# DeepGraphLearning/ultra_torchdrug

Hardware: AMD Instinct MI355X
Metric: edges aggregated/sec, FB15k237-shaped 6L x 64d rspmm Bellman-Ford (predict: the reference's 18 rspmm layers per batch as 6 relation-graph + 6 entity-graph launches, tails and heads in one pass) (higher is better)
Workload: dtype f32

## Files before the change

### include/ultra_rspmm.h

```cpp
#ifndef ULTRA_RSPMM_H
#define ULTRA_RSPMM_H

#include <stddef.h>
#include <stdint.h>

#ifdef __cplusplus
extern "C" {
#endif
#pragma GCC visibility push(default)

#define ULTRA_RSPMM_ABI_VERSION 8

enum ultra_sum_op { ULTRA_SUM_ADD = 0, ULTRA_SUM_MIN = 1, ULTRA_SUM_MAX = 2 };
enum ultra_mul_op { ULTRA_MUL_MUL = 0, ULTRA_MUL_ADD = 1 };

enum ultra_status {
    ULTRA_OK = 0,
    ULTRA_ERR_BAD_OP = 1,
    ULTRA_ERR_BAD_SHAPE = 2,
    ULTRA_ERR_NULL_POINTER = 3,
    ULTRA_ERR_WORKSPACE = 4,
    ULTRA_ERR_HIP = 5,
    ULTRA_ERR_NO_DEVICE = 6,
    ULTRA_ERR_ABI = 7
// ... 99 lines not shown
int ultra_rspmm_backward_accumulate_f32(const ultra_segments *by_src_host, const ultra_segments *by_rel_host,
                                        const float *relation, const float *input, const float *output,
                                        const float *output_grad, const float *d_input_add, float *d_input,
                                        float *d_relation, void *workspace, size_t workspace_bytes, int64_t n_src,
                                        int64_t n_dst, int64_t n_rel, int64_t F, int sum_op, int mul_op, void *stream);

int ultra_rspmm_backward_active_f32(const ultra_segments *by_src, const ultra_segments *by_rel, const float *relation,
                                    const float *input, const float *output_grad, const float *d_input_add, float *d_input,
                                    float *d_relation, void *workspace, size_t workspace_bytes, int64_t n_src, int64_t n_dst,
                                    int64_t n_rel, int64_t F, int mul_op, const uint32_t *dst_active_bits, int64_t active_words,
                                    const int32_t *src_active_node, void *stream);
int ultra_node_bitmap(const int64_t *t_index, int64_t n_batch, int64_t per_row, int64_t n_node, uint32_t *bits, void *stream);

int ultra_rspmm_drelation_boundary_f32(const ultra_segments *by_rel, const int32_t *items, int64_t n_items, const int32_t *src_ptr,
                                       const int32_t *src_relpos, const int32_t *src_node, const float *input,
                                       const float *output_grad, float *d_relation, void *workspace, size_t workspace_bytes,
                                       int64_t n_src, int64_t n_rel, int64_t F, void *stream);

int ultra_rspmm_backward_weight_f32(const ultra_segments *fwd_host, const float *relation, const float *input,
                                    const float *output, const float *output_grad, float *d_weight,
                                    int64_t n_rel, int64_t F, int sum_op, int mul_op, void *stream);

int ultra_rspmm_rotate_forward_f32(const ultra_segments *fwd_host, const float *relation, const float *input,
                                   const float *add_rows, const int32_t *boundary_node, const float *boundary_value,
                                   float *out, void *workspace, size_t workspace_bytes, int64_t n_src, int64_t n_rel,
                                   int64_t F, int64_t block, int sum_op, void *stream);

int ultra_rspmm_rotate_backward_f32(const ultra_segments *by_src_host, const ultra_segments *by_rel_host,
                                    const float *relation, const float *input, const float *output,
                                    const float *output_grad, float *d_input, float *d_relation, void *workspace,
                                    size_t workspace_bytes, int64_t n_src, int64_t n_dst, int64_t n_rel, int64_t F,
                                    int64_t block, int sum_op, void *stream);

int ultra_beam_search_step_f32(const int32_t *row_ptr, const int32_t *src, const float *edge_grad, const float *input,
                               int64_t n_node, int64_t n_edges, int64_t tail, int64_t K, float *distance,
                               int32_t *back_edge, int32_t *back_rank, void *stream);


int ultra_combine_forward_f32(const float *input, const float *update, const float *weight, const float *bias,
                              const float *ln_weight, const float *ln_bias, float ln_eps, int relu, int shortcut,
                              float *out, float *z_out, int64_t rows, int64_t dim, void *stream);

int ultra_combine_forward_boundary_f32(const int32_t *boundary_node, const float *boundary_value, int64_t n_query,
                                       const float *update, const float *weight, const float *bias, const float *ln_weight,
                                       const float *ln_bias, float ln_eps, int relu, int shortcut, float *out, int64_t rows,
                                       int64_t dim, void *stream);


int ultra_combine_backward_waves(int device, int64_t rows, int *n_ln_waves, int *n_wgrad_waves);
int ultra_combine_backward_f32(const float *input, const float *update, const float *weight, const float *bias,
                               const float *ln_weight, const float *ln_bias, float ln_eps, int relu,
                               const float *grad_out, float *d_z, float *d_ln_weight_partial,
                               float *d_ln_bias_partial, float *d_weight_partial, float *d_bias_partial, int64_t rows,
                               int64_t dim, void *stream);

int ultra_combine_dxdu_f32(const float *d_z, const float *weight, const float *grad_out, float *d_input, float *d_update,
                           int64_t rows, int64_t dim, void *stream);


int ultra_combine_backward_fused_waves(int device, int64_t rows, int *n_waves);
int ultra_combine_backward_fused_f32(const float *input, const float *update, const float *weight, const float *bias,
                                     const float *ln_weight, const float *ln_bias, float ln_eps, int relu, int shortcut,
                                     const float *grad_out, const float *z, float *d_input, float *d_update, float *d_weight,
                                     float *d_bias, float *d_ln_weight, float *d_ln_bias, float *partial_workspace,
                                     size_t workspace_bytes, const int32_t *tile_list, int64_t n_list, int64_t rows, int64_t dim, void *stream);


int ultra_linear_forward_f32(const float *input, const float *weight, const float *bias, float *out, int64_t rows,
                             int64_t in_dim, int64_t out_dim, int relu, void *stream);


int ultra_score_forward_f32(const float *hidden, const float *query, const float *w1, const float *b1, const float *w2,
                            const float *b2, float *query_bias, float *out, int64_t n_node, int64_t batch, void *stream);

int ultra_relation_project_f32(const float *relation, int64_t stride_b, int64_t stride_r, const float *const *w1,
                               const float *const *b1, const float *const *w2, const float *const *b2, float *const *out,
                               int64_t n_layers, int64_t batch, int64_t repeat, int64_t n_rel, int64_t dim, void *stream);

int ultra_prepare_queries(const int64_t *batch, const float *rel_rep, int64_t stride_b, int64_t stride_r, int64_t n_batch,
                          int64_t n_rel2, int64_t n_base_rel, int64_t *anchor, int32_t *anchor32, int64_t *relation,
                          float *query, void *stream);

int ultra_relation_stack_inputs(const float *const *weights, int64_t n_layers, int64_t n_rel, int64_t n_query,
                                const int64_t *h_index, int64_t h_stride, float *tables, float *ones, int32_t *node32,
                                void *stream);

int ultra_candidate_tiles(const int64_t *t_index, int64_t n_batch, int64_t per_row, int64_t n_query, int64_t n_rows, int32_t *out,
                          void *stream);

int ultra_gather_boundary_rows_f32(const float *rows, const int32_t *node, int64_t n_query, float *out, void *stream);

int ultra_score_rows_forward_f32(const float *hidden, const float *query, const int64_t *t_index, const float *w1, const float *b1,
                                 const float *w2, const float *b2, float *h, float *in_rows, float *score, int64_t n_batch,
                                 int64_t per_row, void *stream);
int ultra_score_rows_backward_f32(const float *hidden, const float *query, const int64_t *t_index, const float *w1, const float *w2,
                                  const float *h, const float *in_rows, const float *grad, float *d_pre, float *partial,
                                  float *d_hidden, float *d_query, float *d_w1, float *d_b1, float *d_w2, float *d_b2,
                                  int64_t n_node, int64_t n_batch, int64_t per_row, void *stream);

int ultra_statistics_blocks(int64_t n_a);
int ultra_statistics_f32(const float *a, int64_t n_a, const float *b, int64_t n_b, int64_t b_repeat, double *partials,
                         float *out, void *stream);

int ultra_bce_adversarial_f32(const float *pred, int64_t rows, int64_t cols, float temperature, float *loss_rows,
                              float *dpred, void *stream);

int ultra_relation_project_backward_blocks(int device, int64_t batch, int64_t n_rel, int64_t n_layers, int64_t *blocks);
int ultra_relation_project_backward_f32(const float *relation, const float *const *w1, const float *const *b1,
                                        const float *const *w2, const float *const *grad, float *d_relation_layers,
                                        float *const *d_w1, float *const *d_b1, float *const *d_w2, float *const *d_b2,
                                        void *workspace, size_t workspace_bytes, int64_t n_layers, int64_t batch,
                                        int64_t n_rel, int64_t dim, void *stream);

int ultra_filtered_rank(const float *pred, int64_t n_query, int64_t n_cand, int64_t row_stride, const int64_t *target,
                        const int32_t *filt_ptr, const int32_t *filt_node, int64_t *rank, void *stream);


int ultra_filtered_rank_keys(const float *pred, int64_t n_query, int64_t n_cand, int64_t row_stride, const int64_t *target,
                             int64_t target_stride, const int64_t *keys, int64_t n_keys, const int64_t *anchor,
                             const int64_t *rel, int64_t index_stride, int64_t n_rel, int64_t *rank, int64_t rank_stride,
                             void *stream);
int ultra_strict_negative(const int64_t *keys, int64_t n_keys, const int64_t *anchor, const int64_t *rel, int64_t n_query,
                          int64_t n_rel, int64_t n_node, const float *rand, int64_t n_sample, int64_t *out, void *stream);
int ultra_edge_removal_weights(const ultra_segments *fwd, const ultra_segments *by_src, const ultra_segments *by_rel,
                               const int64_t *h, const int64_t *t, const int64_t *r, int64_t n_pattern,
                               int64_t n_base_rel, float *w_fwd, float *w_src, float *w_rel, int64_t slack, void *stream);
int ultra_edge_removal_marks(const ultra_segments *fwd, const ultra_segments *by_src, const ultra_segments *by_rel,
                             const int64_t *h, const int64_t *t, const int64_t *r, int64_t n_pattern, int64_t n_base_rel,
                             float *w_fwd, float *w_src, float *w_rel, int64_t slack, uint32_t *words_fwd, uint32_t *words_src,
                             uint32_t *words_rel, int64_t n_node, void *stream);


size_t ultra_relcsr_coalesce_temp_bytes(int64_t n_edges);
int ultra_relcsr_coalesce(const int64_t *row, const int64_t *col, const int64_t *rel, const float *weight,
                          int64_t n_edges, int64_t n_rows, int64_t n_cols, int64_t n_rel, int32_t *out_row,
                          int32_t *out_col, int32_t *out_rel, float *out_weight, int64_t *edge_of_input,
                          int64_t *n_unique_host, int *unit_weight_host, void *temp, size_t temp_bytes, void *stream);
size_t ultra_relcsr_plan_temp_bytes(int64_t n_edges, int64_t n_rows, int64_t piece_len);
int ultra_relcsr_plan(const int32_t *row, const int32_t *node_a, const int32_t *rel, int64_t n_edges, int64_t n_rows,
                      int64_t n_node_a, int64_t n_rel, int is_relation_plan, int wide_ids, int balance,
                      int64_t chunk_edges, int64_t chunk_rows, int64_t piece_len, int32_t *chunks,
                      int64_t cap_chunks, int32_t *long_rows, int64_t cap_long, int32_t *packed,
                      int64_t packed_slack, int64_t *counts_host, void *temp, size_t temp_bytes, void *stream);

size_t ultra_relcsr_dense_bytes(int64_t n_rows, int64_t n_cols, int kind);
int ultra_relcsr_dense(const ultra_segments *plan, int64_t n_rows, int64_t n_cols, int kind, uint32_t *dense, void *stream);

int ultra_dense_layer_supported(const ultra_segments *fwd, int64_t n_query);
int ultra_dense_layer_forward_f32(const ultra_segments *fwd, const float *relation, const float *input,
                                  const int32_t *boundary_node, const float *boundary_value, int64_t n_query, const float *weight,
                                  const float *bias, const float *ln_weight, const float *ln_bias, float ln_eps, int relu,
                                  int shortcut, float *out, void *stream);

int ultra_layer_forward_supported(const ultra_segments *fwd, int64_t n_query, int64_t n_rel);
int ultra_layer_forward_f32(const ultra_segments *fwd, const float *relation, const float *input, const int32_t *boundary_node,
                            const float *boundary_value, int64_t n_query, const float *weight, const float *bias,
                            const float *ln_weight, const float *ln_bias, float ln_eps, int relu, int shortcut, float *out,
                            int64_t n_rel, void *stream);

int ultra_second_layer_sources(const int32_t *col, int64_t n_edges, int64_t slack, const int32_t *row_list, const int32_t *list_count,
                               int64_t list_len, int64_t n_query, int64_t n_node, uint32_t *bitmap, int32_t *c_node,
                               int32_t *sources, void *stream);
int ultra_layer_forward_sources_f32(const ultra_segments *fwd, const int32_t *sources, const float *relation, const float *input,
                                    const int32_t *boundary_node, const float *boundary_value, int64_t n_query, const float *weight,
                                    const float *bias, const float *ln_weight, const float *ln_bias, float ln_eps, int relu,
                                    int shortcut, float *out, int64_t n_rel, void *stream);

int ultra_layer_score_supported(const ultra_segments *fwd, int64_t n_query, int64_t n_rel);
int ultra_layer_score_forward_f32(const ultra_segments *fwd, const float *relation, const float *input, const int32_t *boundary_node,
                                  const float *boundary_value, int64_t n_query, const float *weight, const float *bias,
                                  const float *ln_weight, const float *ln_bias, float ln_eps, int relu, int shortcut,
                                  const float *query, const float *w1, const float *b1, const float *w2, const float *b2,
                                  float *qbias, float *score, int64_t n_rel, void *stream);

int ultra_relation_graph_marks(const int32_t *head_ptr, const int32_t *head_rel, const int32_t *tail_ptr, const int32_t *tail_rel,
                               int64_t n_node, int64_t n_rel, uint8_t *marks, void *stream);

int ultra_calibrate_gather_f32(const float *table, int64_t n_rows, const int32_t *index, int64_t n_index, float *out,
                               int64_t *n_waves_host, void *stream);

#pragma GCC visibility pop
#ifdef __cplusplus
}
#endif
#endif
```

### ultra_torchdrug_amd/_lib.py

```python
import ctypes
import os

_HERE = os.path.dirname(os.path.abspath(__file__))
LIB_PATH = os.environ.get("ULTRA_RSPMM_LIB") or os.path.join(_HERE, "libultra_rspmm.so")
ABI_VERSION = 8

SUM_OPS = {"add": 0, "min": 1, "max": 2}
MUL_OPS = {"mul": 0, "add": 1}


class UltraSegments(ctypes.Structure):
    _fields_ = [
        ("struct_bytes", ctypes.c_uint32),
        ("abi_version", ctypes.c_uint32),
        ("n_rows", ctypes.c_int64),
        ("n_edges", ctypes.c_int64),
        ("row", ctypes.c_void_p),
        ("node_a", ctypes.c_void_p),
        ("node_b", ctypes.c_void_p),
        ("rel", ctypes.c_void_p),
        ("weight", ctypes.c_void_p),
        ("n_chunks", ctypes.c_int64),
        ("chunks", ctypes.c_void_p),
        ("n_long_rows", ctypes.c_int64),
        ("long_rows", ctypes.c_void_p),
        ("n_pieces", ctypes.c_int64),
        ("piece_len", ctypes.c_int64),
        ("packed", ctypes.c_void_p),
        ("packed_src_shift", ctypes.c_int64),
        ("n_hot", ctypes.c_int64),
        ("hot_nodes", ctypes.c_void_p),
        ("row_ptr", ctypes.c_void_p),
        ("dense", ctypes.c_void_p),
        ("dense_rows", ctypes.c_int64),
        ("dense_cols", ctypes.c_int64),
        ("packed_dead", ctypes.c_void_p),
    ]

    def __init__(self, *args, **kwargs):
        super().__init__(*args, **kwargs)
        if not self.struct_bytes:
            self.struct_bytes = ctypes.sizeof(type(self))
        if not self.abi_version:
            self.abi_version = ABI_VERSION


EXPORTS = (
    "ultra_rspmm_abi_version",
    "ultra_segments_bytes",
    "ultra_rspmm_status_string",
    "ultra_rspmm_last_hip_error",
    "ultra_rspmm_device_info",
    "ultra_rspmm_profile_next",
    "ultra_rspmm_event_create",
    "ultra_rspmm_event_destroy",
    "ultra_rspmm_event_elapsed_ms",
    "ultra_rspmm_force_general_path",
    "ultra_rspmm_reserve_cus",
    "ultra_rspmm_workspace_bytes",
    "ultra_rspmm_forward_f32",
    "ultra_rspmm_fwd_f32",
    "ultra_rspmm_forward_boundary_f32",
    "ultra_rspmm_frontier_f32",
    "ultra_first_layer_sparse_supported",
    "ultra_first_layer_sparse_f32",
    "ultra_rspmm_backward_boundary_rows_f32",
    "ultra_rspmm_backward_boundary_rows_workspace",
    "ultra_rspmm_backward_f32",
    "ultra_rspmm_backward_accumulate_f32",
    "ultra_rspmm_backward_weight_f32",
    "ultra_beam_search_step_f32",
    "ultra_rspmm_backward_active_f32",
    "ultra_node_bitmap",
    "ultra_rspmm_drelation_boundary_f32",
    "ultra_combine_forward_f32",
    "ultra_combine_forward_boundary_f32",
    "ultra_combine_backward_waves",
    "ultra_combine_backward_f32",
    "ultra_combine_dxdu_f32",
    "ultra_combine_backward_fused_waves",
    "ultra_combine_backward_fused_f32",
    "ultra_linear_forward_f32",
    "ultra_score_forward_f32",
    "ultra_relation_project_f32",
    "ultra_relation_project_backward_blocks",
    "ultra_relation_project_backward_f32",
    "ultra_filtered_rank",
    "ultra_filtered_rank_keys",
    "ultra_strict_negative",
    "ultra_edge_removal_weights",
    "ultra_edge_removal_marks",
    "ultra_prepare_queries",
    "ultra_relation_stack_inputs",
    "ultra_statistics_blocks",
    "ultra_statistics_f32",
    "ultra_bce_adversarial_f32",
    "ultra_candidate_tiles",
    "ultra_score_rows_forward_f32",
    "ultra_score_rows_backward_f32",
    "ultra_gather_boundary_rows_f32",
    "ultra_relcsr_coalesce_temp_bytes",
    "ultra_relcsr_coalesce",
    "ultra_relcsr_plan_temp_bytes",
    "ultra_relcsr_plan",
    "ultra_relcsr_dense_bytes",
    "ultra_relcsr_dense",
    "ultra_relation_graph_marks",
    "ultra_calibrate_gather_f32",
    "ultra_first_layer_sparse_train_f32",
    "ultra_first_layer_epilogue_backward_workspace",
    "ultra_first_layer_epilogue_backward_f32",
    "ultra_column_sum_blocks",
    "ultra_column_sum_f32",
    "ultra_dense_layer_supported",
    "ultra_dense_layer_forward_f32",
    "ultra_layer_forward_supported",
    "ultra_layer_forward_f32",
    "ultra_second_layer_sources",
    "ultra_layer_forward_sources_f32",
    "ultra_layer_score_supported",
    "ultra_layer_score_forward_f32",
    "ultra_rspmm_rotate_forward_f32",
    "ultra_rspmm_rotate_backward_f32",
)

_lib = None


class UltraLibraryError(RuntimeError):
    pass


def load():
    global _lib
    if _lib is not None:
        return _lib
    if not os.path.exists(LIB_PATH):
        raise UltraLibraryError(
            "%s not found: build it with `make -C ultra_torchdrug_amd/csrc` (hipcc --offload-arch=gfx950) or "
            "`python -c 'import __graft_entry__ as g; g.build()'`. There is no CPU/PyTorch fallback." % LIB_PATH)
    try:
        lib = ctypes.CDLL(LIB_PATH)
    except OSError as err:
        raise UltraLibraryError("cannot load %s: %s" % (LIB_PATH, err)) from err
    missing = [name for name in EXPORTS if not hasattr(lib, name)]
    if missing:
        raise UltraLibraryError("%s lacks symbols %s" % (LIB_PATH, missing))

    vp, i64, i32, sz = ctypes.c_void_p, ctypes.c_int64, ctypes.c_int, ctypes.c_size_t
    seg = ctypes.POINTER(UltraSegments)
    lib.ultra_rspmm_abi_version.restype = i32
    lib.ultra_rspmm_abi_version.argtypes = []
    lib.ultra_layer_forward_supported.restype = i32
    lib.ultra_layer_forward_supported.argtypes = [seg, i64, i64]
    lib.ultra_layer_forward_f32.restype = i32
    lib.ultra_layer_forward_f32.argtypes = [seg, vp, vp, vp, vp, i64, vp, vp, vp, vp, ctypes.c_float, i32, i32, vp, i64, vp]
    lib.ultra_second_layer_sources.restype = i32
    lib.ultra_second_layer_sources.argtypes = [vp, i64, i64, vp, vp, i64, i64, i64, vp, vp, vp, vp]
    lib.ultra_layer_forward_sources_f32.restype = i32
    lib.ultra_layer_forward_sources_f32.argtypes = [seg, vp, vp, vp, vp, vp, i64, vp, vp, vp, vp, ctypes.c_float, i32, i32, vp, i64, vp]
    lib.ultra_layer_score_supported.restype = i32
    lib.ultra_layer_score_supported.argtypes = [seg, i64, i64]
    lib.ultra_layer_score_forward_f32.restype = i32
    lib.ultra_layer_score_forward_f32.argtypes = [seg, vp, vp, vp, vp, i64, vp, vp, vp, vp, ctypes.c_float, i32, i32, vp, vp, vp, vp,
                                                  vp, vp, vp, i64, vp]
    lib.ultra_relation_graph_marks.restype = i32
    lib.ultra_relation_graph_marks.argtypes = [vp, vp, vp, vp, i64, i64, vp, vp]
    lib.ultra_segments_bytes.restype = sz
    lib.ultra_segments_bytes.argtypes = []
    lib.ultra_rspmm_status_string.restype = ctypes.c_char_p
    lib.ultra_rspmm_status_string.argtypes = [i32]
    lib.ultra_rspmm_last_hip_error.restype = i32
    lib.ultra_rspmm_last_hip_error.argtypes = []
    lib.ultra_rspmm_device_info.restype = i32
    lib.ultra_rspmm_device_info.argtypes = [i32, ctypes.POINTER(i32), ctypes.POINTER(i32), ctypes.c_char_p, sz]
    lib.ultra_rspmm_profile_next.restype = i32
    lib.ultra_rspmm_profile_next.argtypes = [vp, vp]
    lib.ultra_rspmm_event_create.restype = i32
    lib.ultra_rspmm_event_create.argtypes = [ctypes.POINTER(vp)]
    lib.ultra_rspmm_event_destroy.restype = i32
    lib.ultra_rspmm_event_destroy.argtypes = [vp]
    lib.ultra_rspmm_event_elapsed_ms.restype = i32
    lib.ultra_rspmm_event_elapsed_ms.argtypes = [vp, vp, ctypes.POINTER(ctypes.c_float)]
    lib.ultra_rspmm_force_general_path.restype = i32
    lib.ultra_rspmm_force_general_path.argtypes = [i32]
    lib.ultra_rspmm_reserve_cus.restype = i32
    lib.ultra_rspmm_reserve_cus.argtypes = [i32]
    lib.ultra_rspmm_workspace_bytes.restype = sz
    lib.ultra_rspmm_workspace_bytes.argtypes = [seg, i64]
    lib.ultra_rspmm_forward_f32.restype = i32
    lib.ultra_rspmm_forward_f32.argtypes = [seg, vp, vp, vp, vp, vp, sz, i64, i64, i64, i32, i32, vp]
    lib.ultra_rspmm_fwd_f32.restype = i32
    lib.ultra_rspmm_fwd_f32.argtypes = [vp, vp, vp, vp, vp, vp, vp, i64, i64, i64, i64, i32, i32, vp]
    lib.ultra_rspmm_forward_boundary_f32.restype = i32
    lib.ultra_rspmm_forward_boundary_f32.argtypes = [seg, vp, vp, vp, vp, i64, vp, vp, sz, i64, i64, i64, i32, i32, vp]
    lib.ultra_rspmm_backward_boundary_rows_f32.restype = i32
    lib.ultra_rspmm_backward_boundary_rows_f32.argtypes = [seg, vp, vp, vp, vp, vp, vp, sz, i64, i64, i64, i32, vp]
    lib.ultra_rspmm_backward_boundary_rows_workspace.restype = sz
    lib.ultra_rspmm_backward_boundary_rows_workspace.argtypes = [i64]
    lib.ultra_rspmm_frontier_f32.restype = i32
    lib.ultra_rspmm_frontier_f32.argtypes = [seg, vp, vp, vp, vp, vp, i64, vp, i64, i64, i64, vp]
    lib.ultra_first_layer_sparse_supported.restype = i32
    lib.ultra_first_layer_sparse_supported.argtypes = [i64, i64, i64]
    lib.ultra_first_layer_sparse_f32.restype = i32
    lib.ultra_first_layer_sparse_f32.argtypes = [seg, vp, vp, vp, vp, vp, vp, i64, vp, vp, vp, vp, ctypes.c_float, i32, i32, vp, vp, i64, i64,
                                                 vp, i64, i64, vp]
    lib.ultra_rspmm_backward_f32.restype = i32
    lib.ultra_rspmm_backward_f32.argtypes = [seg, seg, vp, vp, vp, vp, vp, vp, vp, sz, i64, i64, i64, i64, i32, i32, vp]
    lib.ultra_rspmm_backward_accumulate_f32.restype = i32
    lib.ultra_rspmm_backward_accumulate_f32.argtypes = [seg, seg, vp, vp, vp, vp, vp, vp, vp, vp, sz, i64, i64, i64, i64, i32,
                                                        i32, vp]
    lib.ultra_rspmm_backward_active_f32.restype = i32
    lib.ultra_rspmm_backward_active_f32.argtypes = [seg, seg, vp, vp, vp, vp, vp, vp, vp, sz, i64, i64, i64, i64, i32, vp, i64, vp, vp]
    lib.ultra_node_bitmap.restype = i32
    lib.ultra_node_bitmap.argtypes = [vp, i64, i64, i64, vp, vp]
    lib.ultra_rspmm_drelation_boundary_f32.restype = i32
    lib.ultra_rspmm_drelation_boundary_f32.argtypes = [seg, vp, i64, vp, vp, vp, vp, vp, vp, vp, sz, i64, i64, i64, vp]
    lib.ultra_rspmm_backward_weight_f32.restype = i32
    lib.ultra_rspmm_backward_weight_f32.argtypes = [seg, vp, vp, vp, vp, vp, i64, i64, i32, i32, vp]
    lib.ultra_beam_search_step_f32.restype = i32
    lib.ultra_beam_search_step_f32.argtypes = [vp, vp, vp, vp, i64, i64, i64, i64, vp, vp, vp, vp]
    lib.ultra_combine_forward_f32.restype = i32
    lib.ultra_combine_forward_f32.argtypes = [vp, vp, vp, vp, vp, vp, ctypes.c_float, i32, i32, vp, vp, i64, i64, vp]
    lib.ultra_combine_forward_boundary_f32.restype = i32
    lib.ultra_combine_forward_boundary_f32.argtypes = [vp, vp, i64, vp, vp, vp, vp, vp, ctypes.c_float, i32, i32, vp, i64, i64, vp]
    lib.ultra_prepare_queries.restype = i32
    lib.ultra_prepare_queries.argtypes = [vp, vp, i64, i64, i64, i64, i64, vp, vp, vp, vp, vp]
    lib.ultra_statistics_blocks.restype = i32
    lib.ultra_statistics_blocks.argtypes = [i64]
    lib.ultra_statistics_f32.restype = i32
    lib.ultra_statistics_f32.argtypes = [vp, i64, vp, i64, i64, vp, vp, vp]
    lib.ultra_gather_boundary_rows_f32.restype = i32
    lib.ultra_gather_boundary_rows_f32.argtypes = [vp, vp, i64, vp, vp]
    lib.ultra_score_rows_forward_f32.restype = i32
    lib.ultra_score_rows_forward_f32.argtypes = [vp] * 10 + [i64, i64, vp]
    lib.ultra_score_rows_backward_f32.restype = i32
    lib.ultra_score_rows_backward_f32.argtypes = [vp] * 16 + [i64, i64, i64, vp]
    lib.ultra_candidate_tiles.restype = i32
    lib.ultra_candidate_tiles.argtypes = [vp, i64, i64, i64, i64, vp, vp]
    lib.ultra_bce_adversarial_f32.restype = i32
    lib.ultra_bce_adversarial_f32.argtypes = [vp, i64, i64, ctypes.c_float, vp, vp, vp]
    lib.ultra_relation_stack_inputs.restype = i32
    lib.ultra_relation_stack_inputs.argtypes = [vp, i64, i64, i64, vp, i64, vp, vp, vp, vp]
    lib.ultra_combine_backward_waves.restype = i32
    lib.ultra_combine_backward_waves.argtypes = [i32, i64, ctypes.POINTER(i32), ctypes.POINTER(i32)]
    lib.ultra_combine_backward_f32.restype = i32
    lib.ultra_combine_backward_f32.argtypes = [vp, vp, vp, vp, vp, vp, ctypes.c_float, i32, vp, vp, vp, vp, vp, vp, i64, i64, vp]
    lib.ultra_combine_dxdu_f32.restype = i32
    lib.ultra_combine_dxdu_f32.argtypes = [vp, vp, vp, vp, vp, i64, i64, vp]
    lib.ultra_combine_backward_fused_waves.restype = i32
    lib.ultra_combine_backward_fused_waves.argtypes = [i32, i64, ctypes.POINTER(i32)]
    lib.ultra_combine_backward_fused_f32.restype = i32
    lib.ultra_combine_backward_fused_f32.argtypes = [vp, vp, vp, vp, vp, vp, ctypes.c_float, i32, i32, vp, vp, vp, vp, vp, vp, vp,
                                                     vp, vp, sz, vp, i64, i64, i64, vp]
    lib.ultra_linear_forward_f32.restype = i32
    lib.ultra_linear_forward_f32.argtypes = [vp, vp, vp, vp, i64, i64, i64, i32, vp]
    lib.ultra_score_forward_f32.restype = i32
    lib.ultra_score_forward_f32.argtypes = [vp, vp, vp, vp, vp, vp, vp, vp, i64, i64, vp]
    lib.ultra_relation_project_f32.restype = i32
    lib.ultra_relation_project_f32.argtypes = [vp, i64, i64, vp, vp, vp, vp, vp, i64, i64, i64, i64, i64, vp]
    lib.ultra_relation_project_backward_blocks.restype = i32
    lib.ultra_relation_project_backward_blocks.argtypes = [i32, i64, i64, i64, vp]
    lib.ultra_relation_project_backward_f32.restype = i32
    lib.ultra_relation_project_backward_f32.argtypes = [vp, vp, vp, vp, vp, vp, vp, vp, vp, vp, vp, sz, i64, i64, i64, i64, vp]
    lib.ultra_filtered_rank.restype = i32
    lib.ultra_filtered_rank.argtypes = [vp, i64, i64, i64, vp, vp, vp, vp, vp]
    lib.ultra_filtered_rank_keys.restype = i32
    lib.ultra_filtered_rank_keys.argtypes = [vp, i64, i64, i64, vp, i64, vp, i64, vp, vp, i64, i64, vp, i64, vp]
    lib.ultra_strict_negative.restype = i32
    lib.ultra_strict_negative.argtypes = [vp, i64, vp, vp, i64, i64, i64, vp, i64, vp, vp]
    lib.ultra_edge_removal_weights.restype = i32
    lib.ultra_edge_removal_weights.argtypes = [seg, seg, seg, vp, vp, vp, i64, i64, vp, vp, vp, i64, vp]
    lib.ultra_edge_removal_marks.restype = i32
    lib.ultra_edge_removal_marks.argtypes = [seg, seg, seg, vp, vp, vp, i64, i64, vp, vp, vp, i64, vp, vp, vp, i64, vp]
    lib.ultra_relcsr_coalesce_temp_bytes.restype = sz
    lib.ultra_relcsr_coalesce_temp_bytes.argtypes = [i64]
    lib.ultra_relcsr_coalesce.restype = i32
    lib.ultra_relcsr_coalesce.argtypes = [vp, vp, vp, vp, i64, i64, i64, i64, vp, vp, vp, vp, vp,
                                          ctypes.POINTER(i64), ctypes.POINTER(i32), vp, sz, vp]
    lib.ultra_relcsr_plan_temp_bytes.restype = sz
    lib.ultra_relcsr_plan_temp_bytes.argtypes = [i64, i64, i64]
    lib.ultra_relcsr_plan.restype = i32
    lib.ultra_relcsr_plan.argtypes = [vp, vp, vp, i64, i64, i64, i64, i32, i32, i32, i64, i64, i64, vp, i64, vp, i64,
                                      vp, i64, ctypes.POINTER(i64), vp, sz, vp]
    lib.ultra_relcsr_dense_bytes.restype = sz
    lib.ultra_relcsr_dense_bytes.argtypes = [i64, i64, i32]
    lib.ultra_relcsr_dense.restype = i32
    lib.ultra_relcsr_dense.argtypes = [seg, i64, i64, i32, vp, vp]
    lib.ultra_first_layer_sparse_train_f32.restype = i32
    lib.ultra_first_layer_sparse_train_f32.argtypes = [seg, vp, vp, vp, vp, vp, vp, i64, vp, vp, vp, vp, ctypes.c_float, i32, i32, vp, vp,
                                                       vp, i64, i64, vp, i64, i64, vp]
    lib.ultra_first_layer_epilogue_backward_workspace.restype = sz
    lib.ultra_first_layer_epilogue_backward_workspace.argtypes = [i32, i64]
    lib.ultra_first_layer_epilogue_backward_f32.restype = i32
    lib.ultra_first_layer_epilogue_backward_f32.argtypes = [vp, vp, vp, vp, vp, i64, vp, vp, vp, vp, ctypes.c_float, i32, i32, vp, vp, vp,
                                                            vp, vp, vp, vp, sz, i64, vp]
    lib.ultra_column_sum_blocks.restype = i32
    lib.ultra_column_sum_blocks.argtypes = []
    lib.ultra_column_sum_f32.restype = i32
    lib.ultra_column_sum_f32.argtypes = [vp, i64, vp, vp, vp, vp]
    lib.ultra_dense_layer_supported.restype = i32
    lib.ultra_dense_layer_supported.argtypes = [seg, i64]
    lib.ultra_dense_layer_forward_f32.restype = i32
    lib.ultra_dense_layer_forward_f32.argtypes = [seg, vp, vp, vp, vp, i64, vp, vp, vp, vp, ctypes.c_float, i32, i32, vp, vp]
    lib.ultra_calibrate_gather_f32.restype = i32
    lib.ultra_calibrate_gather_f32.argtypes = [vp, i64, vp, i64, vp, ctypes.POINTER(i64), vp]
    lib.ultra_rspmm_rotate_forward_f32.restype = i32
    lib.ultra_rspmm_rotate_forward_f32.argtypes = [seg, vp, vp, vp, vp, vp, vp, vp, sz, i64, i64, i64, i64, i32, vp]
    lib.ultra_rspmm_rotate_backward_f32.restype = i32
    lib.ultra_rspmm_rotate_backward_f32.argtypes = [seg, seg, vp, vp, vp, vp, vp, vp, vp, sz, i64, i64, i64, i64, i64, i32, vp]
    if lib.ultra_rspmm_abi_version() != ABI_VERSION:
        raise UltraLibraryError("ABI mismatch: library %d, binding %d" % (lib.ultra_rspmm_abi_version(), ABI_VERSION))
    if lib.ultra_segments_bytes() != ctypes.sizeof(UltraSegments):
        raise UltraLibraryError("struct ultra_segments: library %d bytes, binding %d bytes"
                                % (lib.ultra_segments_bytes(), ctypes.sizeof(UltraSegments)))
    _lib = lib
    return lib


def check(status):
    if status != 0:
        lib = load()
        msg = lib.ultra_rspmm_status_string(status).decode()
        if status == 5:
            msg += " [hipError_t=%d]" % lib.ultra_rspmm_last_hip_error()
        raise RuntimeError("libultra_rspmm: %s" % msg)


def device_info(device=0):
    lib = load()
    n_cu, lds = ctypes.c_int(0), ctypes.c_int(0)
    arch = ctypes.create_string_buffer(64)
    check(lib.ultra_rspmm_device_info(int(device), ctypes.byref(n_cu), ctypes.byref(lds), arch, 64))
    return {"n_cu": n_cu.value, "lds_bytes": lds.value, "arch": arch.value.decode()}
```

### ultra_torchdrug_amd/csrc/relgraph_dense.h

```cpp
#ifndef ULTRA_RELGRAPH_DENSE_H
#define ULTRA_RELGRAPH_DENSE_H

#include <hip/hip_runtime.h>

#include <cstddef>
#include <cstdint>

#include "ultra_rspmm.h"

namespace ultra_detail {

struct DenseCall {
    const ultra_segments *seg;
    int kind, sum_op, mul_op;
    const float *relation;
    const float *input;
    const float *grad;
    const float *add_rows;
    const int32_t *bnode;
    const float *bvec;
    int bdim;
    float *out;
    void *workspace;
    size_t workspace_bytes;
    int64_t gather_rows, gather2_rows, n_rel, F;
};

int persistent_cus(int *n_cu);
bool wide_groups_forced();

bool dense_applies(const DenseCall &call);
int dense_launch(const DenseCall &call, hipStream_t stream);

}

#endif
```

### ultra_torchdrug_amd/csrc/relgraph_dense.hip

```cpp
#include <hip/hip_runtime.h>

#include <cstdint>

#include "relgraph_dense.h"
#include "ultra_rspmm.h"

extern thread_local int ultra_detail_last_hip_error;

namespace {

#define HIP_TRY(expr)                                   \
    do {                                                \
        hipError_t _e = (expr);                         \
        if (_e != hipSuccess) {                         \
            ultra_detail_last_hip_error = (int)_e;      \
            (void)hipGetLastError();                    \
            return ULTRA_ERR_HIP;                       \
        }                                               \
    } while (0)

constexpr int kXcd = 8;
__device__ __forceinline__ int uniform(int v) { return __builtin_amdgcn_readfirstlane(v); }
using ultra_detail::DenseCall;
constexpr int KIND_FWD = 0, KIND_DX = 1, KIND_DREL = 2;

typedef float dn4 __attribute__((ext_vector_type(4)));
constexpr int kDnU = 8;
constexpr int kDnQ = 4;
constexpr int kDnWaves = 4;

struct DenseParams {
    const uint32_t *adj;
    const float *relation;
    const float *gather;
    const float *grad;
    const float *add_rows;
    const int32_t *bnode;
    const float *bvec;
    int bdim;
    float *out;
    long long F;
    int n_rows, n_cols, n_vt, n_ct;
    int cols_pad;
    int n_items, per_xcd;
};

__device__ __forceinline__ bool dense_item(const DenseParams &p, int &vt, int &ct) {
    const int j = blockIdx.x / kXcd;
    const int item = (blockIdx.x % kXcd) * p.per_xcd + j;
    if (j >= p.per_xcd || item >= p.n_items) return false;
    const int n_qb = (p.n_ct + kDnWaves - 1) / kDnWaves;
    vt = item / n_qb;
    ct = (item - vt * n_qb) * kDnWaves + uniform((int)(threadIdx.x >> 6));
    return ct < p.n_ct;
}

#ifndef ULTRA_DN_VARIANT
#define ULTRA_DN_VARIANT 0
#endif

template <int B>
__device__ __forceinline__ float entry(uint32_t word) {
#if ULTRA_DN_VARIANT >= 1
    return 1.0f;
#else
    return (float)((word >> (8 * B)) & 0xffu);
#endif
}

template <int MUL, bool HAS_REL>
__device__ __forceinline__ dn4 dense_rows_sum(const DenseParams &p, const int vt, const int ct, const int lane) {
    const int i = lane & 15, kq = lane >> 4;
    const long long F = p.F;
    const int col = ct * 16 + i;
    float relv = 0.0f;
    if constexpr (HAS_REL) relv = p.relation[(long long)kq * F + col];
    const uint32_t row_bytes = (uint32_t)F * 4u;
    const __amdgpu_buffer_rsrc_t rsrc_x =
        __builtin_amdgcn_make_buffer_rsrc(const_cast<float *>(p.gather), 0, (int)((uint32_t)p.n_cols * row_bytes), 0x00020000);
    const uint32_t slab_words = (uint32_t)(p.cols_pad / 4) * 64u;
    const __amdgpu_buffer_rsrc_t rsrc_a = __builtin_amdgcn_make_buffer_rsrc(
        const_cast<uint32_t *>(p.adj + (long long)vt * slab_words), 0, (int)((slab_words + 4u * 64u) * 4u), 0x00020000);
    const uint32_t voff_x0 = (uint32_t)kq * row_bytes + (uint32_t)col * 4u, voff_a = (uint32_t)lane * 4u;
    const int pick[4] = {4 * i, 4 * (i + 16), 4 * (i + 32), 4 * (i + 48)};

    auto load = [&](int u0, float (&x)[2], uint32_t (&a)[2]) {
#pragma unroll
        for (int h = 0; h < 2; ++h) {
            x[h] = __builtin_bit_cast(float, __builtin_amdgcn_raw_buffer_load_b32(rsrc_x, voff_x0 + (uint32_t)(u0 + 4 * h) * row_bytes, 0, 0));
            a[h] = __builtin_amdgcn_raw_buffer_load_b32(rsrc_a, voff_a, (uint32_t)(u0 / 4 + h) * 256u, 0);
        }
    };
    auto spread = [&](const float (&x)[2], float (&xs)[kDnU]) {
#pragma unroll
        for (int j = 0; j < kDnU; ++j) {
#if ULTRA_DN_VARIANT >= 4
            xs[j] = 1.5f;
#elif ULTRA_DN_VARIANT >= 2
            xs[j] = x[j >> 2];
#else
            xs[j] = __builtin_bit_cast(float, __builtin_amdgcn_ds_bpermute(pick[j & 3], __builtin_bit_cast(int, x[j >> 2])));
#endif
        }
    };
    dn4 acc = {0.0f, 0.0f, 0.0f, 0.0f};
    auto message = [&](float xv) -> float {
#if ULTRA_DN_VARIANT >= 3
        return xv;
#endif
        if constexpr (!HAS_REL) return xv;
        return (MUL == ULTRA_MUL_MUL) ? relv * xv : relv + xv;
    };
    auto compute = [&](const float (&xs)[kDnU], const uint32_t (&a)[2]) {
        acc = __builtin_amdgcn_mfma_f32_16x16x4f32(entry<0>(a[0]), message(xs[0]), acc, 0, 0, 0);
        acc = __builtin_amdgcn_mfma_f32_16x16x4f32(entry<1>(a[0]), message(xs[1]), acc, 0, 0, 0);
        acc = __builtin_amdgcn_mfma_f32_16x16x4f32(entry<2>(a[0]), message(xs[2]), acc, 0, 0, 0);
        acc = __builtin_amdgcn_mfma_f32_16x16x4f32(entry<3>(a[0]), message(xs[3]), acc, 0, 0, 0);
        acc = __builtin_amdgcn_mfma_f32_16x16x4f32(entry<0>(a[1]), message(xs[4]), acc, 0, 0, 0);
        acc = __builtin_amdgcn_mfma_f32_16x16x4f32(entry<1>(a[1]), message(xs[5]), acc, 0, 0, 0);
        acc = __builtin_amdgcn_mfma_f32_16x16x4f32(entry<2>(a[1]), message(xs[6]), acc, 0, 0, 0);
        acc = __builtin_amdgcn_mfma_f32_16x16x4f32(entry<3>(a[1]), message(xs[7]), acc, 0, 0, 0);
    };
    float x0[2], x1[2], s0[kDnU], s1[kDnU];
    uint32_t a0[2], a1[2], c0[2], c1[2];
    load(0, x0, a0);
    load(kDnU, x1, a1);
    spread(x0, s0);
    c0[0] = a0[0]; c0[1] = a0[1];
    for (int u0 = 0; u0 < p.cols_pad; u0 += 2 * kDnU) {
        load(u0 + 2 * kDnU, x0, a0);
        spread(x1, s1);
        c1[0] = a1[0]; c1[1] = a1[1];
        compute(s0, c0);
        load(u0 + 3 * kDnU, x1, a1);
        spread(x0, s0);
        c0[0] = a0[0]; c0[1] = a0[1];
        compute(s1, c1);
    }
    return acc;
}

template <int MUL, bool HAS_REL>
__global__ __launch_bounds__(kDnWaves * 64) void dense_rows_kernel(const DenseParams p) {
    int vt, ct;
    if (!dense_item(p, vt, ct)) return;
    const int lane = threadIdx.x & 63;
    const int i = lane & 15, kq = lane >> 4;
    const long long F = p.F;
    const int col = ct * 16 + i;
    const dn4 acc = dense_rows_sum<MUL, HAS_REL>(p, vt, ct, lane);

    int b_node = -1;
    float b_val = 0.0f;
    if (p.add_rows == nullptr && p.bnode != nullptr) {
        b_node = p.bnode[col / p.bdim];
        b_val = p.bvec[col];
    }
#pragma unroll
    for (int r = 0; r < 4; ++r) {
        const int row = vt * 16 + 4 * kq + r;
        if (row < p.n_rows) {
            float v = acc[r];
            if (p.add_rows != nullptr) v = v + p.add_rows[(long long)row * F + col];
            else if (p.bnode != nullptr) v = v + (row == b_node ? b_val : 0.0f);
            p.out[(long long)row * F + col] = v;
        }
    }
}

struct DenseLayerParams {
    DenseParams d;
    const float *weight;
    const float *bias, *gamma, *beta;
    float eps;
    int relu, shortcut;
    float *out;
};
constexpr int kDlStride = 68;

__global__ __launch_bounds__(kDnWaves * 64) void dense_layer_kernel(const DenseLayerParams q) {
    const DenseParams &p = q.d;
    __shared__ __attribute__((aligned(16))) float t_in[16 * kDlStride], t_up[16 * kDlStride], t_z[16 * kDlStride];
    int vt, ct;
    if (!dense_item(p, vt, ct)) return;
    const int lane = threadIdx.x & 63, wave = ct & 3;
    const int i = lane & 15, kq = lane >> 4;
    const long long F = p.F;
    const int col = ct * 16 + i;
    float wf[32];
    {
        const float *wrow = q.weight + (long long)(16 * wave + i) * 128 + 64 * (kq & 1) + (kq >> 1);
#pragma unroll
        for (int j = 0; j < 32; ++j) wf[j] = wrow[2 * j];
    }
    const float bias = q.bias[16 * wave + i];
    {
        const int row = vt * 16 + 4 * wave + kq;
        dn4 v = {0.0f, 0.0f, 0.0f, 0.0f};
        if (row < p.n_rows) v = *reinterpret_cast<const dn4 *>(p.gather + (long long)row * F + (ct & ~3) * 16 + 4 * i);
        *reinterpret_cast<dn4 *>(t_in + (4 * wave + kq) * kDlStride + 4 * i) = v;
    }
    const dn4 acc = dense_rows_sum<ULTRA_MUL_MUL, true>(p, vt, ct, lane);
    {
        const int b_node = p.bnode[col / 64];
        const float b_val = p.bvec[col];
#pragma unroll
        for (int r = 0; r < 4; ++r) {
            const int row = vt * 16 + 4 * kq + r;
            t_up[(4 * kq + r) * kDlStride + 16 * wave + i] = acc[r] + (row == b_node ? b_val : 0.0f);
        }
    }
    __syncthreads();
    dn4 z = {bias, bias, bias, bias};
    {
        const float *src = ((kq & 1) ? t_up : t_in) + i * kDlStride + (kq >> 1);
#pragma unroll
        for (int j = 0; j < 32; ++j) z = __builtin_amdgcn_mfma_f32_16x16x4f32(src[2 * j], wf[j], z, 0, 0, 0);
    }
#pragma unroll
    for (int r = 0; r < 4; ++r) t_z[(4 * kq + r) * kDlStride + 16 * wave + i] = z[r];
    __syncthreads();
    const int lrow = 4 * wave + kq;
    const float *zr = t_z + lrow * kDlStride;
    dn4 v = *reinterpret_cast<const dn4 *>(zr + 4 * i);
    if (q.gamma != nullptr) {
        const int half = (i >> 3) & 1;
        float s = 0.0f;
        if ((i & 7) == 0)
            for (int c = 0; c < 32; ++c) s = s + zr[32 * half + c];
        const float s0 = __shfl(s, 16 * kq, 64), s1 = __shfl(s, 16 * kq + 8, 64);
        const float mean = (s0 + s1) * (1.0f / 64.0f);
        float ss = 0.0f;
        if ((i & 7) == 0)
            for (int c = 0; c < 32; ++c) { const float dlt = zr[32 * half + c] - mean; ss = ss + dlt * dlt; }
        const float q0 = __shfl(ss, 16 * kq, 64), q1 = __shfl(ss, 16 * kq + 8, 64);
        const float var = (q0 + q1) * (1.0f / 64.0f);
        const float inv = 1.0f / sqrtf(var + q.eps);
        const dn4 g = *reinterpret_cast<const dn4 *>(q.gamma + 4 * i), b = *reinterpret_cast<const dn4 *>(q.beta + 4 * i);
        v.x = ((v.x - mean) * inv) * g.x + b.x; v.y = ((v.y - mean) * inv) * g.y + b.y;
        v.z = ((v.z - mean) * inv) * g.z + b.z; v.w = ((v.w - mean) * inv) * g.w + b.w;
    }
    if (q.relu) {
        v.x = !(v.x <= 0.0f) ? v.x : 0.0f; v.y = !(v.y <= 0.0f) ? v.y : 0.0f; v.z = !(v.z <= 0.0f) ? v.z : 0.0f; v.w = !(v.w <= 0.0f) ? v.w : 0.0f;
    }
    if (q.shortcut) {
        const dn4 x = *reinterpret_cast<const dn4 *>(t_in + lrow * kDlStride + 4 * i);
        v.x = v.x + x.x; v.y = v.y + x.y; v.z = v.z + x.z; v.w = v.w + x.w;
    }
    const int row = vt * 16 + lrow;
    if (row < p.n_rows) *reinterpret_cast<dn4 *>(q.out + (long long)row * F + (ct & ~3) * 16 + 4 * i) = v;
}

__global__ __launch_bounds__(kDnWaves * 64) void dense_drel_kernel(const DenseParams p) {
    int vt, ct;
    if (!dense_item(p, vt, ct)) return;
    const int lane = threadIdx.x & 63;
    const int i = lane & 15, kq = lane >> 4;
    const long long F = p.F;
    const int col = ct * 16 + i;
    const uint32_t row_bytes = (uint32_t)F * 4u;
    const __amdgpu_buffer_rsrc_t rsrc_x =
        __builtin_amdgcn_make_buffer_rsrc(const_cast<float *>(p.gather), 0, (int)((uint32_t)p.n_cols * row_bytes), 0x00020000);
    const uint32_t n_h = (uint32_t)p.cols_pad / 16u;
    const __amdgpu_buffer_rsrc_t rsrc_a = __builtin_amdgcn_make_buffer_rsrc(
        const_cast<uint32_t *>(p.adj), 0, (int)((4u * (uint32_t)p.n_vt * n_h + 2u) * 256u), 0x00020000);
    const uint32_t voff_a = (uint32_t)lane * 4u;
    uint32_t base_t[4];
#pragma unroll
    for (int t = 0; t < 4; ++t) base_t[t] = ((uint32_t)(t * p.n_vt + vt) * n_h) * 256u;
    const uint32_t voff_x0 = (uint32_t)kq * row_bytes + (uint32_t)col * 4u;

    auto load = [&](int h, float (&x)[kDnQ], uint32_t (&a)[4]) {
#pragma unroll
        for (int j = 0; j < kDnQ; ++j) {
            x[j] = __builtin_bit_cast(float, __builtin_amdgcn_raw_buffer_load_b32(rsrc_x, voff_x0 + (uint32_t)(16 * h + 4 * j) * row_bytes, 0, 0));
#if ULTRA_DN_VARIANT >= 4
            x[j] = 1.5f;
#endif
        }
#pragma unroll
        for (int t = 0; t < 4; ++t) a[t] = __builtin_amdgcn_raw_buffer_load_b32(rsrc_a, voff_a, base_t[t] + (uint32_t)h * 256u, 0);
    };
    dn4 acc[4];
#pragma unroll
    for (int t = 0; t < 4; ++t) acc[t] = dn4{0.0f, 0.0f, 0.0f, 0.0f};
    auto compute = [&](const float (&x)[kDnQ], const uint32_t (&a)[4]) {
#pragma unroll
        for (int t = 0; t < 4; ++t) {
            acc[t] = __builtin_amdgcn_mfma_f32_16x16x4f32(entry<0>(a[t]), x[0], acc[t], 0, 0, 0);
            acc[t] = __builtin_amdgcn_mfma_f32_16x16x4f32(entry<1>(a[t]), x[1], acc[t], 0, 0, 0);
            acc[t] = __builtin_amdgcn_mfma_f32_16x16x4f32(entry<2>(a[t]), x[2], acc[t], 0, 0, 0);
            acc[t] = __builtin_amdgcn_mfma_f32_16x16x4f32(entry<3>(a[t]), x[3], acc[t], 0, 0, 0);
        }
    };
    float xa[kDnQ], xb[kDnQ];
    uint32_t aa[4], ab[4];
    load(0, xa, aa);
    const int n_blocks = p.cols_pad / 16;
    for (int h = 0; h < n_blocks; h += 2) {
        load(h + 1, xb, ab);
        compute(xa, aa);
        load(h + 2, xa, aa);
        compute(xb, ab);
    }

    float gv[4];
#pragma unroll
    for (int r = 0; r < 4; ++r) {
        const int row = vt * 16 + 4 * kq + r;
        gv[r] = row < p.n_rows ? p.grad[(long long)row * F + col] : 0.0f;
    }
#pragma unroll
    for (int t = 0; t < 4; ++t) {
        const float q = ((gv[0] * acc[t][0] + gv[1] * acc[t][1]) + gv[2] * acc[t][2]) + gv[3] * acc[t][3];
        const int qi = __builtin_bit_cast(int, q);
        const float q0 = __builtin_bit_cast(float, __builtin_amdgcn_ds_bpermute(4 * i, qi));
        const float q1 = __builtin_bit_cast(float, __builtin_amdgcn_ds_bpermute(4 * (i + 16), qi));
        const float q2 = __builtin_bit_cast(float, __builtin_amdgcn_ds_bpermute(4 * (i + 32), qi));
        const float q3 = __builtin_bit_cast(float, __builtin_amdgcn_ds_bpermute(4 * (i + 48), qi));
        const float tile = ((q0 + q1) + q2) + q3;
        if (kq == 0) p.out[((long long)vt * 4 + t) * F + col] = tile;
    }
}

__global__ __launch_bounds__(256) void dense_drel_reduce_kernel(const float *tiles, float *d_relation, long long F, int n_vt) {
    const long long idx = (long long)blockIdx.x * blockDim.x + threadIdx.x;
    if (idx >= 4 * F) return;
    const long long t = idx / F, c = idx - t * F;
    float acc = 0.0f;
    for (int v0 = 0; v0 < n_vt; v0 += 16) {
        float part[16];
#pragma unroll
        for (int j = 0; j < 16; ++j) part[j] = tiles[((long long)min(v0 + j, n_vt - 1) * 4 + t) * F + c];
#pragma unroll
        for (int j = 0; j < 16; ++j)
            if (v0 + j < n_vt) acc = acc + part[j];
    }
    d_relation[idx] = acc;
}

__global__ __launch_bounds__(256) void dense_build_kernel(const int32_t *row, const int32_t *node_a, const int32_t *node_b,
                                                          long long n_edges, int kind, int n_vt, int cols_pad, uint8_t *dense,
                                                          const int32_t *rel) {
    const long long e = (long long)blockIdx.x * blockDim.x + threadIdx.x;
    if (e >= n_edges) return;
    long long idx;
    if (kind == 0) {
        const int v = row[e], u = node_a[e], t = rel[e];
        if (t < 0 || t >= 4) return;
        idx = ((((long long)(v >> 4) * (cols_pad / 4) + (u >> 2)) * 4 + t) * 16 + (v & 15)) * 4 + (u & 3);
    } else {
        const int t = row[e], u = node_a[e], v = node_b[e];
        if (t < 0 || t >= 4) return;
        idx = (((((long long)t * n_vt + (v >> 4)) * (cols_pad / 16) + (u >> 4)) * 4 + (u & 3)) * 16 + (v & 15)) * 4 + ((u >> 2) & 3);
    }
    dense[idx] = 1;
}

__global__ __launch_bounds__(256) void dense_zero_kernel(uint32_t *dense, long long n_words) {
    const long long k = (long long)blockIdx.x * blockDim.x + threadIdx.x;
    if (k < n_words) dense[k] = 0u;
}

inline int dense_cols_pad(long long n_cols, int kind) {
    const int round = kind == 0 ? 2 * kDnU : 8 * kDnQ;
    return (int)((n_cols + round - 1) / round * round);
}
inline long long dense_slack_bytes(int kind) { return kind == 0 ? 2 * kDnU * 64 : 2 * 256; }

}

namespace ultra_detail {

bool dense_applies(const DenseCall &c) {
    const ultra_segments *seg = c.seg;
    if (seg->dense == nullptr || seg->weight != nullptr || c.sum_op != ULTRA_SUM_ADD || c.n_rel != 4) return false;
    if (c.F % 16 != 0 || c.F * 4 >= (1LL << 24)) return false;
    if (seg->dense_cols != c.gather_rows || c.gather_rows * c.F * 4 >= (1LL << 31)) return false;
    if (c.kind == KIND_DREL) {
        if (c.mul_op != ULTRA_MUL_MUL || seg->n_rows != 4 || seg->dense_rows != c.gather2_rows) return false;
        const long long n_vt = (seg->dense_rows + 15) / 16;
        if (c.workspace == nullptr || c.workspace_bytes < (size_t)(n_vt * 4 * c.F) * sizeof(float)) return false;
    } else {
        if (seg->dense_rows != seg->n_rows) return false;
        if (c.kind == KIND_FWD && c.add_rows == nullptr && c.bnode != nullptr && c.bdim <= 0) return false;
    }
    return true;
}

int dense_launch(const DenseCall &c, hipStream_t stream) {
    const ultra_segments *seg = c.seg;
    const long long F = c.F;
    DenseParams q{};
    q.adj = seg->dense;
    q.relation = c.relation;
    q.gather = (c.kind == KIND_DX) ? c.grad : c.input;
    q.grad = c.grad;
    q.add_rows = (c.kind == KIND_DREL) ? nullptr : c.add_rows;
    q.bnode = (c.kind == KIND_FWD) ? c.bnode : nullptr;
    q.bvec = c.bvec;
    q.bdim = c.bdim;
    q.out = (c.kind == KIND_DREL) ? static_cast<float *>(c.workspace) : c.out;
    q.F = F;
    q.n_rows = (int)seg->dense_rows;
    q.n_cols = (int)seg->dense_cols;
    q.n_vt = (int)((seg->dense_rows + 15) / 16);
    q.n_ct = (int)(F / 16);
    q.cols_pad = dense_cols_pad(seg->dense_cols, c.kind == KIND_DREL ? 1 : 0);
    const int n_qb = (q.n_ct + kDnWaves - 1) / kDnWaves;
    q.n_items = q.n_vt * n_qb;
    q.per_xcd = (q.n_items + kXcd - 1) / kXcd;
    const dim3 grid((unsigned)(q.per_xcd * kXcd)), block(kDnWaves * 64);
    if (c.kind == KIND_DREL) {
        hipLaunchKernelGGL(dense_drel_kernel, grid, block, 0, stream, q);
        HIP_TRY(hipGetLastError());
        const long long n = 4 * F;
        hipLaunchKernelGGL(dense_drel_reduce_kernel, dim3((unsigned)((n + 255) / 256)), dim3(256), 0, stream,
                           static_cast<const float *>(c.workspace), c.out, F, q.n_vt);
    } else if (c.kind == KIND_FWD) {
        if (c.mul_op == ULTRA_MUL_MUL) hipLaunchKernelGGL((dense_rows_kernel<ULTRA_MUL_MUL, true>), grid, block, 0, stream, q);
        else hipLaunchKernelGGL((dense_rows_kernel<ULTRA_MUL_ADD, true>), grid, block, 0, stream, q);
    } else {
        if (c.mul_op == ULTRA_MUL_MUL) hipLaunchKernelGGL((dense_rows_kernel<ULTRA_MUL_MUL, true>), grid, block, 0, stream, q);
        else hipLaunchKernelGGL((dense_rows_kernel<ULTRA_MUL_ADD, false>), grid, block, 0, stream, q);
    }
    HIP_TRY(hipGetLastError());
    return ULTRA_OK;
}

}

namespace {

constexpr int kCalRowsPerWave = 2048;
typedef uint32_t cu4 __attribute__((ext_vector_type(4)));

__global__ __launch_bounds__(512) void calibrate_gather_kernel(const float *table, uint32_t table_bytes, const int32_t *index,
                                                               long long n_waves, float *out) {
    const int lane = threadIdx.x & 63;
    const int q = lane >> 4, j = lane & 15;
    const long long wave = ((long long)blockIdx.x * blockDim.x + threadIdx.x) >> 6;
    if (wave >= n_waves) return;
    const int32_t *mine = index + wave * kCalRowsPerWave;
    const __amdgpu_buffer_rsrc_t rsrc = __builtin_amdgcn_make_buffer_rsrc(const_cast<float *>(table), 0, (int)table_bytes, 0x00020000);
    float acc = 0.0f;
    int ids = mine[lane & 31];
    for (int k = 0; k < kCalRowsPerWave; k += 32) {
        const int nxt = (k + 32 < kCalRowsPerWave) ? mine[k + 32 + (lane & 31)] : 0;
        cu4 v[8];
#pragma unroll
        for (int u = 0; u < 8; ++u) {
            const uint32_t row = (uint32_t)__builtin_amdgcn_ds_bpermute(4 * (u * 4 + q), ids);
            v[u] = __builtin_amdgcn_raw_buffer_load_b128(rsrc, row * 256u + (uint32_t)j * 16u, 0, 0);
        }
#pragma unroll
        for (int u = 0; u < 8; ++u)
            acc += (__builtin_bit_cast(float, v[u].x) + __builtin_bit_cast(float, v[u].y)) +
                   (__builtin_bit_cast(float, v[u].z) + __builtin_bit_cast(float, v[u].w));
        ids = nxt;
    }
    out[wave * 64 + lane] = acc;
}

}

extern "C" {

size_t ultra_relcsr_dense_bytes(int64_t n_rows, int64_t n_cols, int kind) {
    if (n_rows <= 0 || n_cols <= 0 || (kind != 0 && kind != 1) || n_rows > (1 << 20) || n_cols > (1 << 20)) return 0;
    const long long n_vt = (n_rows + 15) / 16;
    const long long bytes = n_vt * 64 * dense_cols_pad(n_cols, kind) + dense_slack_bytes(kind);
    if (bytes >= (1LL << 31)) return 0;
    return (size_t)bytes;
}

int ultra_relcsr_dense(const ultra_segments *plan, int64_t n_rows, int64_t n_cols, int kind, uint32_t *dense, void *stream) {
    if (plan == nullptr) return ULTRA_ERR_NULL_POINTER;
    if (plan->struct_bytes != (uint32_t)sizeof(ultra_segments) || plan->abi_version != (uint32_t)ULTRA_RSPMM_ABI_VERSION) return ULTRA_ERR_ABI;
    if (plan->n_edges < 0 || plan->n_edges > 0x7fffffffLL) return ULTRA_ERR_BAD_SHAPE;
    if (plan->n_edges > 0 && (plan->row == nullptr || plan->node_a == nullptr || plan->rel == nullptr)) return ULTRA_ERR_NULL_POINTER;
    const size_t bytes = ultra_relcsr_dense_bytes(n_rows, n_cols, kind);
    if (bytes == 0) return ULTRA_ERR_BAD_SHAPE;
    if (dense == nullptr) return ULTRA_ERR_NULL_POINTER;
    if (plan->weight != nullptr) return ULTRA_ERR_BAD_SHAPE;
    if (kind == 0 && plan->n_rows != n_rows) return ULTRA_ERR_BAD_SHAPE;
    if (kind == 1 && (plan->n_rows != 4 || (plan->n_edges > 0 && plan->node_b == nullptr))) return ULTRA_ERR_BAD_SHAPE;
    hipStream_t s = static_cast<hipStream_t>(stream);
    const long long n_words = (long long)(bytes / 4);
    hipLaunchKernelGGL(dense_zero_kernel, dim3((unsigned)((n_words + 255) / 256)), dim3(256), 0, s, dense, n_words);
    HIP_TRY(hipGetLastError());
    if (plan->n_edges > 0) {
        hipLaunchKernelGGL(dense_build_kernel, dim3((unsigned)((plan->n_edges + 255) / 256)), dim3(256), 0, s, plan->row,
                           plan->node_a, plan->node_b, (long long)plan->n_edges, kind, (int)((n_rows + 15) / 16),
                           dense_cols_pad(n_cols, kind), reinterpret_cast<uint8_t *>(dense), plan->rel);
        HIP_TRY(hipGetLastError());
    }
    return ULTRA_OK;
}

int ultra_dense_layer_supported(const ultra_segments *fwd, int64_t n_query) {
    if (fwd == nullptr || fwd->struct_bytes != (uint32_t)sizeof(ultra_segments) || fwd->abi_version != (uint32_t)ULTRA_RSPMM_ABI_VERSION) return 0;
    if (fwd->dense == nullptr || fwd->weight != nullptr || n_query <= 0) return 0;
    if (fwd->dense_rows != fwd->n_rows || fwd->dense_rows != fwd->dense_cols) return 0;
    const long long F = n_query * 64;
    return (F * 4 < (1LL << 24) && fwd->dense_cols * F * 4 < (1LL << 31)) ? 1 : 0;
}

int ultra_dense_layer_forward_f32(const ultra_segments *fwd, const float *relation, const float *input,
                                  const int32_t *boundary_node, const float *boundary_value, int64_t n_query, const float *weight,
                                  const float *bias, const float *ln_weight, const float *ln_bias, float ln_eps, int relu,
                                  int shortcut, float *out, void *stream) {
    if (fwd != nullptr && (fwd->struct_bytes != (uint32_t)sizeof(ultra_segments) || fwd->abi_version != (uint32_t)ULTRA_RSPMM_ABI_VERSION))
        return ULTRA_ERR_ABI;
    if (!ultra_dense_layer_supported(fwd, n_query)) return ULTRA_ERR_BAD_SHAPE;
    if (relation == nullptr || input == nullptr || boundary_node == nullptr || boundary_value == nullptr || weight == nullptr ||
        bias == nullptr || out == nullptr)
        return ULTRA_ERR_NULL_POINTER;
    if (ln_weight != nullptr && ln_bias == nullptr) return ULTRA_ERR_NULL_POINTER;
    if (out == input) return ULTRA_ERR_BAD_SHAPE;
    if ((reinterpret_cast<uintptr_t>(out) | reinterpret_cast<uintptr_t>(input) | reinterpret_cast<uintptr_t>(ln_weight) |
         reinterpret_cast<uintptr_t>(ln_bias)) & 15u)
        return ULTRA_ERR_BAD_SHAPE;
    DenseLayerParams q{};
    DenseParams &d = q.d;
    const long long F = n_query * 64;
    d.adj = fwd->dense; d.relation = relation; d.gather = input; d.bnode = boundary_node; d.bvec = boundary_value; d.bdim = 64;
    d.F = F; d.n_rows = (int)fwd->dense_rows; d.n_cols = (int)fwd->dense_cols; d.n_vt = (int)((fwd->dense_rows + 15) / 16);
    d.n_ct = (int)(F / 16); d.cols_pad = dense_cols_pad(fwd->dense_cols, 0);
    d.n_items = d.n_vt * (d.n_ct / kDnWaves); d.per_xcd = (d.n_items + kXcd - 1) / kXcd;
    q.weight = weight; q.bias = bias; q.gamma = ln_weight; q.beta = ln_bias; q.eps = ln_eps; q.relu = relu; q.shortcut = shortcut;
    q.out = out;
    hipLaunchKernelGGL(dense_layer_kernel, dim3((unsigned)(d.per_xcd * kXcd)), dim3(kDnWaves * 64), 0, static_cast<hipStream_t>(stream), q);
    HIP_TRY(hipGetLastError());
    return ULTRA_OK;
}

int ultra_calibrate_gather_f32(const float *table, int64_t n_rows, const int32_t *index, int64_t n_index, float *out,
                               int64_t *n_waves_host, void *stream) {
    if (n_rows <= 0 || n_index < 0 || n_rows * 256 >= (1LL << 32)) return ULTRA_ERR_BAD_SHAPE;
    const long long n_waves = n_index / kCalRowsPerWave;
    if (n_waves_host != nullptr) *n_waves_host = n_waves;
    if (out == nullptr || n_waves == 0) return ULTRA_OK;
    if (table == nullptr || index == nullptr) return ULTRA_ERR_NULL_POINTER;
    hipLaunchKernelGGL(calibrate_gather_kernel, dim3((unsigned)((n_waves + 7) / 8)), dim3(512), 0, static_cast<hipStream_t>(stream),
                       table, (uint32_t)(n_rows * 256), index, n_waves, out);
    HIP_TRY(hipGetLastError());
    return ULTRA_OK;
}

}
```

### ultra_torchdrug_amd/csrc/rspmm_kernels.hip

```cpp
#include <hip/hip_runtime.h>
#include <type_traits>

#include <algorithm>
#include <cstdint>
#include <cstdlib>
#include <cstring>
#include <mutex>

#include "relgraph_dense.h"
#include "ultra_rspmm.h"

thread_local int ultra_detail_last_hip_error = 0;

namespace {

constexpr int kTile = 64;
#ifndef ULTRA_BLOCK
#define ULTRA_BLOCK 1024
#endif
constexpr int kBlock = ULTRA_BLOCK;
#ifndef ULTRA_UNROLL
#define ULTRA_UNROLL 8
#endif
constexpr int kUnroll = ULTRA_UNROLL;
// ... 663 lines not shown
                const int query = (int)(qq - step * (unsigned)p.rpn);
                const f32x4 zero = {0.0f, 0.0f, 0.0f, 0.0f};
                if constexpr (BND == 1) {
                    const f32x4 v = *reinterpret_cast<const f32x4 *>(bv_lds + query * 64 + c);
                    pa[q] = (node0 + step == (long long)bn_lds[query]) ? v : zero;
                } else {
                    pa[q] = (node0 + step == (long long)p.in_bnode[query]) ? *reinterpret_cast<const f32x4 *>(p.in_bvec + query * 64 + c) : zero;
                }
            }
            pb[q] = *reinterpret_cast<const f32x4 *>(p.update + gr * 64 + c);
        }
    };
    if constexpr (PF) {
        if (wave_global < n_tiles) fetch(wave_global);
    }
    for (long long t = wave_global; t < n_tiles; t += wave_total) {
        const long long row0 = t * kCbRows;
        if constexpr (!PF) fetch(t);
#pragma unroll
        for (int q = 0; q < 8; ++q) {
            const int r = 4 * q + (lane >> 4), c = (lane & 15) * 4;
            *reinterpret_cast<f32x4 *>(tile + r * kCbStride + c) = pa[q];
            *reinterpret_cast<f32x4 *>(tile + r * kCbStride + 64 + c) = pb[q];
        }
        if constexpr (PF) {
            asm volatile("s_waitcnt lgkmcnt(0)" ::: "memory");
            if (t + wave_total < n_tiles) fetch(t + wave_total);
        } else {
            asm volatile("s_waitcnt vmcnt(0) lgkmcnt(0)" ::: "memory");
        }

        f32x16 acc0, acc1;
#pragma unroll
        for (int r = 0; r < 16; ++r) { acc0[r] = bias0; acc1[r] = bias1; }
#pragma unroll
        for (int q = 0; q < 16; ++q) {
            const f32x4 av = *reinterpret_cast<const f32x4 *>(tile + i * kCbStride + 64 * h + 4 * q);
            acc0 = __builtin_amdgcn_mfma_f32_32x32x2f32(av.x, w0[4 * q + 0], acc0, 0, 0, 0);
            acc1 = __builtin_amdgcn_mfma_f32_32x32x2f32(av.x, w1[4 * q + 0], acc1, 0, 0, 0);
            acc0 = __builtin_amdgcn_mfma_f32_32x32x2f32(av.y, w0[4 * q + 1], acc0, 0, 0, 0);
            acc1 = __builtin_amdgcn_mfma_f32_32x32x2f32(av.y, w1[4 * q + 1], acc1, 0, 0, 0);
            acc0 = __builtin_amdgcn_mfma_f32_32x32x2f32(av.z, w0[4 * q + 2], acc0, 0, 0, 0);
            acc1 = __builtin_amdgcn_mfma_f32_32x32x2f32(av.z, w1[4 * q + 2], acc1, 0, 0, 0);
            acc0 = __builtin_amdgcn_mfma_f32_32x32x2f32(av.w, w0[4 * q + 3], acc0, 0, 0, 0);
            acc1 = __builtin_amdgcn_mfma_f32_32x32x2f32(av.w, w1[4 * q + 3], acc1, 0, 0, 0);
        }
        asm volatile("s_waitcnt lgkmcnt(0)" ::: "memory");

#pragma unroll
        for (int r = 0; r < 16; ++r) {
            const int row = (r & 3) + 8 * (r >> 2) + 4 * h;
            tile[row * kCbStride + 64 + i] = acc0[r];
            tile[row * kCbStride + 96 + i] = acc1[r];
        }
        asm volatile("s_waitcnt lgkmcnt(0)" ::: "memory");

        float v[32];
#pragma unroll
        for (int q = 0; q < 8; ++q) {
            const f32x4 d = *reinterpret_cast<const f32x4 *>(tile + ln_row * kCbStride + 64 + 32 * ln_half + 4 * q);
            v[4 * q + 0] = d.x; v[4 * q + 1] = d.y; v[4 * q + 2] = d.z; v[4 * q + 3] = d.w;
            if constexpr (ZOUT) {
                const long long left_z = p.rows - row0;
                const __amdgpu_buffer_rsrc_t rsrc_z = __builtin_amdgcn_make_buffer_rsrc(
                    p.z_out + row0 * 64, 0, (int)(left_z < kCbRows ? left_z : kCbRows) * 256, 0x00020000);
                __builtin_amdgcn_raw_buffer_store_b128(__builtin_bit_cast(qu4, d), rsrc_z, ln_row * 256 + ln_half * 128 + 16 * q, 0, 0);
            }
        }
        if (p.gamma != nullptr) {
            float s = 0.0f;
#pragma unroll
            for (int c = 0; c < 32; ++c) s = s + v[c];
            const float so = __shfl_xor(s, 1, 64);
            const float mean = (ln_half == 0 ? s + so : so + s) * (1.0f / 64.0f);
            float ss = 0.0f;
#pragma unroll
            for (int c = 0; c < 32; ++c) { const float dlt = v[c] - mean; ss = ss + dlt * dlt; }
            const float sso = __shfl_xor(ss, 1, 64);
            const float var = (ln_half == 0 ? ss + sso : sso + ss) * (1.0f / 64.0f);
            const float inv = 1.0f / sqrtf(var + p.eps);
#pragma unroll
            for (int q = 0; q < 8; ++q) {
                const f32x4 gq = *reinterpret_cast<const f32x4 *>(gb + 32 * ln_half + 4 * q);
                const f32x4 bq = *reinterpret_cast<const f32x4 *>(gb + 64 + 32 * ln_half + 4 * q);
                v[4 * q + 0] = ((v[4 * q + 0] - mean) * inv) * gq.x + bq.x;
                v[4 * q + 1] = ((v[4 * q + 1] - mean) * inv) * gq.y + bq.y;
                v[4 * q + 2] = ((v[4 * q + 2] - mean) * inv) * gq.z + bq.z;
                v[4 * q + 3] = ((v[4 * q + 3] - mean) * inv) * gq.w + bq.w;
            }
        }
        if (p.relu) {
#pragma unroll
            for (int c = 0; c < 32; ++c) v[c] = !(v[c] <= 0.0f) ? v[c] : 0.0f;
        }
        if (p.shortcut) {
#pragma unroll
            for (int q = 0; q < 8; ++q) {
                const f32x4 x = *reinterpret_cast<const f32x4 *>(tile + ln_row * kCbStride + 32 * ln_half + 4 * q);
                v[4 * q + 0] = v[4 * q + 0] + x.x; v[4 * q + 1] = v[4 * q + 1] + x.y;
                v[4 * q + 2] = v[4 * q + 2] + x.z; v[4 * q + 3] = v[4 * q + 3] + x.w;
            }
        }
#pragma unroll
        for (int q = 0; q < 8; ++q) {
            f32x4 d;
            d.x = v[4 * q + 0]; d.y = v[4 * q + 1]; d.z = v[4 * q + 2]; d.w = v[4 * q + 3];
            *reinterpret_cast<f32x4 *>(tile + ln_row * kCbStride + 64 + 32 * ln_half + 4 * q) = d;
        }
        asm volatile("s_waitcnt lgkmcnt(0)" ::: "memory");

        if constexpr (BND == 3) {
            if (p.rows * 256 >= (1LL << 32) - 65536) {
#pragma unroll
                for (int q = 0; q < 8; ++q) {
                    const int r = 4 * q + (lane >> 4), c = (lane & 15) * 4;
                    const f32x4 d = *reinterpret_cast<const f32x4 *>(tile + r * kCbStride + 64 + c);
                    if (rid[q] >= 0) *reinterpret_cast<f32x4 *>(p.out + (long long)rid[q] * 64 + c) = d;
                }
                asm volatile("s_waitcnt lgkmcnt(0)" ::: "memory");
                continue;
            }
            const __amdgpu_buffer_rsrc_t rsrc_all = __builtin_amdgcn_make_buffer_rsrc(p.out, 0, (int)(uint32_t)(p.rows * 256), 0x00020000);
#pragma unroll
            for (int q = 0; q < 8; ++q) {
                const int r = 4 * q + (lane >> 4), c = (lane & 15) * 4;
                const f32x4 d = *reinterpret_cast<const f32x4 *>(tile + r * kCbStride + 64 + c);
                const uint32_t off = rid[q] >= 0 ? (uint32_t)rid[q] * 256u + (uint32_t)c * 4u : 0xffffffffu;
                __builtin_amdgcn_raw_buffer_store_b128(__builtin_bit_cast(qu4, d), rsrc_all, off, 0, 0);
            }
            asm volatile("s_waitcnt lgkmcnt(0)" ::: "memory");
            continue;
        }
        const long long left = p.rows - row0;
        const __amdgpu_buffer_rsrc_t rsrc_tile = __builtin_amdgcn_make_buffer_rsrc(
            p.out + row0 * 64, 0, (int)(left < kCbRows ? left : kCbRows) * 256, 0x00020000);
#pragma unroll
        for (int q = 0; q < 8; ++q) {
            const int r = 4 * q + (lane >> 4), c = (lane & 15) * 4;
            const f32x4 d = *reinterpret_cast<const f32x4 *>(tile + r * kCbStride + 64 + c);
            __builtin_amdgcn_raw_buffer_store_b128(__builtin_bit_cast(qu4, d), rsrc_tile, r * 256 + c * 4, 0, 0);
        }
        asm volatile("s_waitcnt lgkmcnt(0)" ::: "memory");
    }
}


thread_local hipEvent_t g_prof_start = nullptr;
thread_local hipEvent_t g_prof_stop = nullptr;
bool g_force_general = false;
bool g_no_x_lds = false;
bool g_no_quad = false;
bool g_wide_groups = false;
bool g_no_dead_words = false;
#ifndef ULTRA_QUAD_U
#define ULTRA_QUAD_U 8
#endif
constexpr int kQuadU = ULTRA_QUAD_U;
#ifndef ULTRA_QUAD_UW
#define ULTRA_QUAD_UW 6
#endif
constexpr int kQuadUW = ULTRA_QUAD_UW;
#ifndef ULTRA_QUAD_UX
#define ULTRA_QUAD_UX 8
#endif
constexpr int kQuadUX = ULTRA_QUAD_UX;

#define HIP_TRY(expr)                                   \
    do {                                                \
        hipError_t _e = (expr);                         \
        if (_e != hipSuccess) {                         \
            ultra_detail_last_hip_error = (int)_e;                 \
            (void)hipGetLastError();                    \
            return ULTRA_ERR_HIP;                       \
        }                                               \
    } while (0)

struct DeviceInfo {
    bool valid = false;
    int n_cu = 0;
    int n_cu_total = 0;
    int lds_bytes = 0;
    char arch[64] = {0};
};
DeviceInfo g_dev[16];
int g_reserve_cus = 0;

int device_info(int device, DeviceInfo **out) {
    if (device < 0 || device >= 16) return ULTRA_ERR_NO_DEVICE;
    DeviceInfo &d = g_dev[device];
    if (!d.valid) {
        hipDeviceProp_t prop;
        HIP_TRY(hipGetDeviceProperties(&prop, device));
        d.n_cu_total = prop.multiProcessorCount;
        d.n_cu = std::max(kXcd, d.n_cu_total - g_reserve_cus);
        d.lds_bytes = (int)prop.maxSharedMemoryPerMultiProcessor;
        std::strncpy(d.arch, prop.gcnArchName, sizeof(d.arch) - 1);
        d.valid = true;
    }
    *out = &d;
    return ULTRA_OK;
}

int gcd_int(int a, int b) {
    while (b) {
        int t = a % b;
        a = b;
        b = t;
    }
    return a;
}

struct LdsAttrTable {
    static constexpr int kSlots = 512;
    const void *kern[kSlots];
    int dev[kSlots];
    int n = 0;
    bool seen(const void *k, int d) const {
        for (int i = 0; i < n; ++i)
            if (kern[i] == k && dev[i] == d) return true;
        return false;
    }
    void add(const void *k, int d) {
        if (n < kSlots) { kern[n] = k; dev[n] = d; ++n; }
    }
};
LdsAttrTable g_lds_attr;
std::mutex g_lds_attr_mutex;

int ensure_lds_attribute(const void *kern, size_t lds) {
    if (lds <= 48 * 1024) return ULTRA_OK;
    int dev = 0;
    HIP_TRY(hipGetDevice(&dev));
    std::lock_guard<std::mutex> lock(g_lds_attr_mutex);
    if (g_lds_attr.seen(kern, dev)) return ULTRA_OK;
    HIP_TRY(hipFuncSetAttribute(kern, hipFuncAttributeMaxDynamicSharedMemorySize, kMaxLdsBytes));
    g_lds_attr.add(kern, dev);
    return ULTRA_OK;
}

template <typename Kern, typename Params>
int launch_with_lds(Kern kern, const Params &p, int grid, size_t lds, hipStream_t stream, int block = kBlock) {
    const int rc = ensure_lds_attribute(reinterpret_cast<const void *>(kern), lds);
    if (rc) return rc;
    hipLaunchKernelGGL(kern, dim3(grid), dim3(block), lds, stream, p);
    HIP_TRY(hipGetLastError());
    return ULTRA_OK;
}

template <int KIND, int SUM, int MUL, bool UNIT_W, bool REL_LDS>
int launch_instance(const KParams &p, int grid, size_t lds, hipStream_t stream) {
    return launch_with_lds(segment_kernel<KIND, SUM, MUL, UNIT_W, REL_LDS>, p, grid, lds, stream);
}

template <int KIND, int SUM, int MUL>
int launch_wl(const KParams &p, bool unit_w, bool rel_lds, int grid, size_t lds, hipStream_t stream) {
    if constexpr (KIND == KIND_DREL) {
        if (unit_w) return launch_instance<KIND, SUM, MUL, true, false>(p, grid, kLdsHeader, stream);
        return launch_instance<KIND, SUM, MUL, false, false>(p, grid, kLdsHeader, stream);
    } else {
        if (unit_w) {
            if (rel_lds) return launch_instance<KIND, SUM, MUL, true, true>(p, grid, lds, stream);
            return launch_instance<KIND, SUM, MUL, true, false>(p, grid, lds, stream);
        }
        if (rel_lds) return launch_instance<KIND, SUM, MUL, false, true>(p, grid, lds, stream);
        return launch_instance<KIND, SUM, MUL, false, false>(p, grid, lds, stream);
    }
}

template <int KIND>
int launch_ops(const KParams &p, int sum_op, int mul_op, bool unit_w, bool rel_lds, int grid, size_t lds,
               hipStream_t stream) {
#define ULTRA_CASE(S, M)                                                    \
    if (sum_op == S && mul_op == M) return launch_wl<KIND, S, M>(p, unit_w, rel_lds, grid, lds, stream);
    ULTRA_CASE(ULTRA_SUM_ADD, ULTRA_MUL_MUL)
    ULTRA_CASE(ULTRA_SUM_ADD, ULTRA_MUL_ADD)
    ULTRA_CASE(ULTRA_SUM_MIN, ULTRA_MUL_MUL)
    ULTRA_CASE(ULTRA_SUM_MIN, ULTRA_MUL_ADD)
    ULTRA_CASE(ULTRA_SUM_MAX, ULTRA_MUL_MUL)
    ULTRA_CASE(ULTRA_SUM_MAX, ULTRA_MUL_ADD)
#undef ULTRA_CASE
    return ULTRA_ERR_BAD_OP;
}

inline bool segments_abi_ok(const ultra_segments *s) {
    return s->struct_bytes == (uint32_t)sizeof(ultra_segments) && s->abi_version == (uint32_t)ULTRA_RSPMM_ABI_VERSION;
}

int check_segments(const ultra_segments *s) {
    if (s == nullptr) return ULTRA_ERR_NULL_POINTER;
    if (!segments_abi_ok(s)) return ULTRA_ERR_ABI;
    if (s->n_rows < 0 || s->n_edges < 0 || s->n_chunks < 0 || s->n_pieces < 0 || s->n_long_rows < 0)
        return ULTRA_ERR_BAD_SHAPE;
    if (s->n_rows > 0x7fffffffLL || s->n_edges > 0x7fffffffLL || s->n_chunks > 0x7fffffffLL) return ULTRA_ERR_BAD_SHAPE;
    if (s->n_edges > 0 && (s->row == nullptr || s->node_a == nullptr || s->rel == nullptr)) return ULTRA_ERR_NULL_POINTER;
    if (s->n_chunks > 0 && s->chunks == nullptr) return ULTRA_ERR_NULL_POINTER;
    if (s->n_long_rows > 0 && s->long_rows == nullptr) return ULTRA_ERR_NULL_POINTER;
    return ULTRA_OK;
}

template <int KIND, int SUM, int MUL>
int launch_packed_w(const PParams &p, bool unit_w, int var, int grid, size_t lds, hipStream_t stream) {
#define ULTRA_VAR(V)                                                                                                  \
    if (var == V) {                                                                                                   \
        constexpr int UN = (V == 2 || V == 3) ? kUnrollBig : kUnroll;                                                 \
        if (unit_w) return launch_with_lds(packed_kernel<KIND, SUM, MUL, true, V, UN>, p, grid, lds, stream);        \
        return launch_with_lds(packed_kernel<KIND, SUM, MUL, false, V, UN>, p, grid, lds, stream);                   \
// ... 248 lines not shown
    }
    bool use_packed = false;
    if (!use_rowgroup) {
        const float *gather = (KIND == KIND_DX) ? p.grad : p.input;
        const unsigned long long gather_bytes = (unsigned long long)gather_rows * (unsigned long long)F * 4ull;
        const unsigned long long gather2_bytes = (unsigned long long)gather2_rows * (unsigned long long)F * 4ull;
        const bool big = seg->packed_src_shift >= 32;
        const bool rel_fits = lds_need <= (size_t)kMaxLdsBytes && n_rel > 0;
        const unsigned long long relation_bytes = (unsigned long long)n_rel * (unsigned long long)F * 4ull;
        const bool lds_ok = (KIND == KIND_DREL) || rel_fits || (big && relation_bytes < 0xffff0000ull && n_rel > 0);
        use_packed = !g_force_general && seg->packed != nullptr && (KIND == KIND_FWD || sum_op == ULTRA_SUM_ADD) &&
                     lds_ok && gather_bytes < 0xffff0000ull && gather2_bytes < 0xffff0000ull &&
                     (unsigned long long)F * 4ull < 0x7fffffffull && (KIND != KIND_DREL || (seg->node_b != nullptr && !big));
        if (use_packed) {
            PParams q{};
            q.meta = seg->packed;
            q.meta2 = reinterpret_cast<const uint32_t *>(big ? seg->node_a : seg->node_b);
            q.weight = seg->weight;
            q.chunks = p.chunks;
            q.relation = p.relation;
            q.gather = gather;
            q.gather2 = p.grad;
            q.add_rows = p.add_rows;
            q.bnode = p.bnode;
            q.bvec = p.bvec;
            q.bdim = p.bdim;
            q.out = p.out;
            q.partial = p.partial;
            q.F = F;
            q.gather_bytes = (uint32_t)gather_bytes;
            q.gather2_bytes = (uint32_t)gather2_bytes;
            q.relation_bytes = (uint32_t)(relation_bytes < 0xffff0000ull ? relation_bytes : 0);
            q.row_bytes = (uint32_t)(F * 4);
            q.src_shift = (uint32_t)seg->packed_src_shift;
            q.rel_mask = big ? 0xffffff00u : ((1u << (seg->packed_src_shift - 8)) - 1u) << 8;
            q.n_chunks = p.n_chunks;
            q.n_rel = p.n_rel;
            q.n_tiles = n_tiles;
            q.split = split;
            q.n_slots = p.n_slots;
            q.blocks_per_label = blocks_per_label;
            const bool needs_rel = (KIND == KIND_FWD) || (KIND == KIND_DX && mul_op == ULTRA_MUL_MUL);
            const size_t lds_x_bytes = (size_t)gather_rows * kTile * sizeof(float);
            int var = 0;
            size_t lds_bytes = needs_rel ? lds_need : 0;
            if (big) {
                var = (needs_rel && !rel_fits) ? 2 : 3;
                if (var == 2) lds_bytes = 0;
            } else if (seg->n_hot > 0) {
                const size_t hot_bytes = (size_t)seg->n_hot * kTile * sizeof(float);
                if (lds_bytes + hot_bytes > (size_t)kMaxLdsBytes) return ULTRA_ERR_BAD_SHAPE;
                var = 4;
                lds_bytes += hot_bytes;
                q.hot_nodes = seg->hot_nodes;
                q.n_hot = (int)seg->n_hot;
            } else if ((KIND != KIND_DREL || mul_op == ULTRA_MUL_MUL) && !g_no_x_lds && gather_rows > 0 &&
                       lds_bytes + lds_x_bytes <= (size_t)kMaxLdsBytes) {
                var = 1;
                lds_bytes += lds_x_bytes;
            }
            q.n_gather_rows = (int)gather_rows;
            auto aligned16 = [](const void *ptr) { return (reinterpret_cast<uintptr_t>(ptr) & 15u) == 0; };
            const unsigned long long meta_bytes = ((unsigned long long)seg->n_edges + 16ull) * 4ull;
            q.meta_bytes = (uint32_t)(meta_bytes < 0xffff0000ull ? meta_bytes : 0);
            q.meta2_bytes = (uint32_t)((unsigned long long)seg->n_edges * 4ull);
            const unsigned long long out_bytes = (unsigned long long)seg->n_rows * (unsigned long long)F * 4ull;
            q.out_bytes = (uint32_t)(out_bytes < 0xffff0000ull ? out_bytes : 0);
            const bool quad = !g_no_quad && (var == 0 || var == 1) && (F % 4) == 0 && q.out_bytes != 0 &&
                              q.meta_bytes != 0 && (unsigned long long)F * 4ull < (1ull << 24) &&
                              (KIND != KIND_DREL || gather2_rows < (1ll << 24)) && aligned16(gather) && aligned16(p.grad) &&
                              aligned16(p.out) && aligned16(p.add_rows) && aligned16(p.partial) && aligned16(p.bvec) &&
                              (p.bnode == nullptr || p.bdim % 4 == 0);
            if (quad) {
                const int slots_per_label = (q.n_slots + kXcd - 1) / kXcd;
                int conc = 1;
                while (!g_no_concurrent_tiles && conc * 2 <= slots_per_label && blocks_per_label % (conc * 2) == 0 &&
                       blocks_per_label / (conc * 2) >= 4)
                    conc *= 2;
                if (const char *force = getenv("ULTRA_CONC")) {
                    const int want = atoi(force);
                    const char *min_rows = getenv("ULTRA_CONC_MIN_ROWS");
                    if (want >= 1 && blocks_per_label % want == 0 && (min_rows == nullptr || gather_rows >= atoll(min_rows)))
                        conc = want;
                }
                q.concurrent = conc;
                size_t act_bytes = 0;
                if (KIND == KIND_DREL && var == 0 && F % kTile == 0) {
                    if (p.act_bits != nullptr && p.act_words > 0 && lds_bytes + (size_t)p.act_words * 4 <= (size_t)kMaxLdsBytes) {
                        q.act_bits = p.act_bits;
                        q.act_words = p.act_words;
                        act_bytes = (size_t)p.act_words * 4;
                    } else if (KIND == KIND_DREL && p.act_node != nullptr && mul_op == ULTRA_MUL_MUL) {
                        q.act_node = p.act_node;
                    }
                }
                const bool dead = seg->packed_dead != nullptr && !g_no_dead_words && var == 0 && q.act_node == nullptr &&
                                  sum_op == ULTRA_SUM_ADD && mul_op == ULTRA_MUL_MUL;
                if (dead) { q.meta = seg->packed_dead; q.weight = nullptr; }
                rc = launch_quad<KIND>(q, sum_op, mul_op, dead || seg->weight == nullptr, var == 1, grid,
                                       kLdsHeader + lds_bytes + act_bytes, stream, dead);
            }
            if (!quad) rc = launch_packed<KIND>(q, sum_op, mul_op, seg->weight == nullptr, var, grid, kLdsHeader + lds_bytes, stream);
            if (rc) return rc;
        }
    }
    if (!use_packed && !use_rowgroup) {
        rc = launch_ops<KIND>(p, sum_op, mul_op, seg->weight == nullptr, rel_lds, grid,
                              kLdsHeader + (rel_lds ? lds_need : 0), stream);
        if (rc) return rc;
    }
    if (ev_stop != nullptr) HIP_TRY(stamp(ev_stop));

    if (seg->n_long_rows > 0) {
        FixParams fp;
        fp.long_rows = seg->long_rows;
        fp.partial = p.partial;
        fp.add_rows = p.add_rows;
        fp.bnode = p.bnode;
        fp.bvec = p.bvec;
        fp.bdim = p.bdim;
        fp.out = p.out;
        fp.F = F;
        fp.n_long = (int)seg->n_long_rows;
        fp.n_tiles = n_tiles;
        const long long waves = (long long)fp.n_long * n_tiles;
        const int fgrid = (int)((waves + 3) / 4);
        const int red = (KIND == KIND_FWD) ? sum_op : ULTRA_SUM_ADD;
        const bool many_pieces = seg->n_pieces >= 128 * seg->n_long_rows;
        if (red == ULTRA_SUM_ADD && many_pieces)
            hipLaunchKernelGGL((fixup_kernel<ULTRA_SUM_ADD, 64>), dim3(fgrid), dim3(256), 0, stream, fp);
        else if (red == ULTRA_SUM_ADD) hipLaunchKernelGGL(fixup_kernel<ULTRA_SUM_ADD>, dim3(fgrid), dim3(256), 0, stream, fp);
        else if (red == ULTRA_SUM_MIN) hipLaunchKernelGGL(fixup_kernel<ULTRA_SUM_MIN>, dim3(fgrid), dim3(256), 0, stream, fp);
        else hipLaunchKernelGGL(fixup_kernel<ULTRA_SUM_MAX>, dim3(fgrid), dim3(256), 0, stream, fp);
        HIP_TRY(hipGetLastError());
    }
    return ULTRA_OK;
}

#include "rotate.inc"

}

namespace ultra_detail {
int persistent_cus(int *n_cu) {
    int dev = 0;
    HIP_TRY(hipGetDevice(&dev));
    DeviceInfo *di = nullptr;
    const int rc = device_info(dev, &di);
    if (rc) return rc;
    *n_cu = di->n_cu;
    return ULTRA_OK;
}
bool wide_groups_forced() { return g_wide_groups; }
}

extern "C" {

int ultra_rspmm_abi_version(void) { return ULTRA_RSPMM_ABI_VERSION; }

size_t ultra_segments_bytes(void) { return sizeof(ultra_segments); }

const char *ultra_rspmm_status_string(int status) {
    switch (status) {
        case ULTRA_OK: return "ok";
        case ULTRA_ERR_BAD_OP: return "unknown sum/mul operator code";
        case ULTRA_ERR_BAD_SHAPE: return "bad shape (negative size, F <= 0 or index range beyond int32)";
        case ULTRA_ERR_NULL_POINTER: return "required pointer is NULL";
        case ULTRA_ERR_WORKSPACE: return "workspace is NULL or smaller than ultra_rspmm_workspace_bytes()";
        case ULTRA_ERR_HIP: return "HIP runtime error (see ultra_rspmm_last_hip_error)";
        case ULTRA_ERR_NO_DEVICE: return "no usable HIP device";
        case ULTRA_ERR_ABI: return "ultra_segments.struct_bytes / abi_version are not this library's (binding written against another include/ultra_rspmm.h)";
        default: return "unknown status";
    }
}

int ultra_rspmm_last_hip_error(void) { return ultra_detail_last_hip_error; }

int ultra_rspmm_reserve_cus(int n) {
    if (n < 0) return ULTRA_ERR_BAD_SHAPE;
    g_reserve_cus = n;
    for (DeviceInfo &d : g_dev)
        if (d.valid) d.n_cu = std::max(kXcd, d.n_cu_total - n);
    return ULTRA_OK;
}

int ultra_rspmm_device_info(int device, int *n_cu, int *lds_bytes, char *arch_host, size_t arch_len) {
    DeviceInfo *di = nullptr;
    int rc = device_info(device, &di);
    if (rc) return rc;
    if (n_cu) *n_cu = di->n_cu_total;
    if (lds_bytes) *lds_bytes = di->lds_bytes;
    if (arch_host && arch_len > 0) {
        std::strncpy(arch_host, di->arch, arch_len - 1);
        arch_host[arch_len - 1] = 0;
    }
    return ULTRA_OK;
}

int ultra_rspmm_force_general_path(int on) {
    g_force_general = (on & 1) != 0;
    g_no_x_lds = (on & 2) != 0;
    g_no_quad = (on & 4) != 0;
    g_no_rowgroup = (on & 8) != 0;
    g_wide_groups = (on & 16) != 0;
    g_no_concurrent_tiles = (on & 32) != 0;
    g_no_dead_words = (on & 128) != 0;
    g_no_dense = (on & 64) != 0;
    return ULTRA_OK;
}

int ultra_rspmm_event_create(void **event) {
    if (event == nullptr) return ULTRA_ERR_NULL_POINTER;
    hipEvent_t e = nullptr;
    HIP_TRY(hipEventCreate(&e));
    *event = e;
    return ULTRA_OK;
}

int ultra_rspmm_event_destroy(void *event) {
    if (event != nullptr) HIP_TRY(hipEventDestroy(static_cast<hipEvent_t>(event)));
    return ULTRA_OK;
}

int ultra_rspmm_event_elapsed_ms(void *start_event, void *stop_event, float *ms_host) {
    if (start_event == nullptr || stop_event == nullptr || ms_host == nullptr) return ULTRA_ERR_NULL_POINTER;
    HIP_TRY(hipEventSynchronize(static_cast<hipEvent_t>(stop_event)));
    HIP_TRY(hipEventElapsedTime(ms_host, static_cast<hipEvent_t>(start_event), static_cast<hipEvent_t>(stop_event)));
    return ULTRA_OK;
}

int ultra_rspmm_profile_next(void *start_event, void *stop_event) {
    g_prof_start = static_cast<hipEvent_t>(start_event);
    g_prof_stop = static_cast<hipEvent_t>(stop_event);
    return ULTRA_OK;
}

size_t ultra_rspmm_workspace_bytes(const ultra_segments *seg, int64_t F) {
    if (seg == nullptr || F <= 0 || !segments_abi_ok(seg)) return 0;
    int64_t rows = seg->n_pieces > 0 ? seg->n_pieces : 0;
    if (seg->dense != nullptr && seg->n_rows == 4 && seg->node_b != nullptr) rows = std::max<int64_t>(rows, 4 * ((seg->dense_rows + 15) / 16));
    return (size_t)rows * (size_t)F * sizeof(float);
}

int ultra_rspmm_forward_f32(const ultra_segments *fwd, const float *relation, const float *input, const float *add_rows,
                            float *out, void *workspace, size_t workspace_bytes, int64_t n_src, int64_t n_rel, int64_t F,
                            int sum_op, int mul_op, void *stream) {
    if (fwd == nullptr) return ULTRA_ERR_NULL_POINTER;
    if (!segments_abi_ok(fwd)) return ULTRA_ERR_ABI;
    if (fwd->n_rows > 0 && out == nullptr) return ULTRA_ERR_NULL_POINTER;
    if (fwd->n_edges > 0 && (relation == nullptr || input == nullptr)) return ULTRA_ERR_NULL_POINTER;
    KParams p{};
    p.relation = relation;
    p.input = input;
    p.add_rows = add_rows;
    p.out = out;
    return run_plan<KIND_FWD>(fwd, p, n_src, 0, n_rel, F, sum_op, mul_op, true, workspace, workspace_bytes,
                              static_cast<hipStream_t>(stream));
}

int ultra_rspmm_fwd_f32(const int32_t *row_ptr, const int32_t *src, const int32_t *rel, const float *w,
                        const float *relation, const float *x, float *out, int64_t N, int64_t E, int64_t R, int64_t F,
                        int sum_op, int mul_op, void *stream) {
    if (N < 0 || E < 0 || R < 0 || F <= 0 || N > 0x7fffffffLL || E > 0x7fffffffLL || (F % 4) != 0) return ULTRA_ERR_BAD_SHAPE;
    if (sum_op < 0 || sum_op > 2 || mul_op < 0 || mul_op > 1) return ULTRA_ERR_BAD_OP;
    if (N == 0) return ULTRA_OK;
    if (row_ptr == nullptr || out == nullptr) return ULTRA_ERR_NULL_POINTER;
    if (E > 0 && (src == nullptr || rel == nullptr || relation == nullptr || x == nullptr)) return ULTRA_ERR_NULL_POINTER;
    if ((reinterpret_cast<uintptr_t>(out) | reinterpret_cast<uintptr_t>(x) | reinterpret_cast<uintptr_t>(relation)) & 15u)
        return ULTRA_ERR_BAD_SHAPE;
    int dev = 0;
    HIP_TRY(hipGetDevice(&dev));
    DeviceInfo *di = nullptr;
    int rc = device_info(dev, &di);
    if (rc) return rc;
    RowGroupParams q{};
    q.row_ptr = row_ptr;
    q.col = src;
    q.rel = rel;
    q.weight = w;
    q.relation = relation;
    q.gather = x;
    q.out = out;
    q.F = F;
    q.n_rows = (int)N;
    q.n_rel = (int)R;
    return launch_rowgroup(q, false, sum_op, mul_op, w == nullptr, N, di->n_cu, static_cast<hipStream_t>(stream));
}

int ultra_rspmm_forward_boundary_f32(const ultra_segments *fwd, const float *relation, const float *input,
                                     const int32_t *boundary_node, const float *boundary_value, int64_t block, float *out,
                                     void *workspace, size_t workspace_bytes, int64_t n_src, int64_t n_rel, int64_t F,
                                     int sum_op, int mul_op, void *stream) {
    if (fwd == nullptr) return ULTRA_ERR_NULL_POINTER;
    if (!segments_abi_ok(fwd)) return ULTRA_ERR_ABI;
    if (boundary_node == nullptr || boundary_value == nullptr) return ULTRA_ERR_NULL_POINTER;
    if (fwd->n_rows > 0 && out == nullptr) return ULTRA_ERR_NULL_POINTER;
    if (fwd->n_edges > 0 && (relation == nullptr || input == nullptr)) return ULTRA_ERR_NULL_POINTER;
    if (block <= 0 || block > 0x7fffffffLL || F <= 0 || F % block != 0) return ULTRA_ERR_BAD_SHAPE;
    KParams p{};
    p.relation = relation;
    p.input = input;
    p.bnode = boundary_node;
    p.bvec = boundary_value;
    p.bdim = (int)block;
    p.out = out;
    return run_plan<KIND_FWD>(fwd, p, n_src, 0, n_rel, F, sum_op, mul_op, true, workspace, workspace_bytes,
                              static_cast<hipStream_t>(stream));
}

int ultra_rspmm_frontier_f32(const ultra_segments *by_src, const int32_t *src_ptr, const int32_t *fwd_rank,
                             const float *relation, const int32_t *boundary_node, const float *boundary_value,
                             int64_t block, float *out, int64_t n_dst, int64_t n_rel, int64_t F, void *stream) {
    int rc = check_segments(by_src);
    if (rc) return rc;
    if (src_ptr == nullptr || boundary_node == nullptr || boundary_value == nullptr) return ULTRA_ERR_NULL_POINTER;
    if (by_src->n_edges > 0 && (fwd_rank == nullptr || relation == nullptr)) return ULTRA_ERR_NULL_POINTER;
    if (block != 64 || F <= 0 || F % 64 != 0 || n_dst < 0 || n_rel < 0 || by_src->piece_len <= 0) return ULTRA_ERR_BAD_SHAPE;
    if (n_dst == 0) return ULTRA_OK;
    if (out == nullptr) return ULTRA_ERR_NULL_POINTER;
    if ((reinterpret_cast<uintptr_t>(out) | reinterpret_cast<uintptr_t>(relation) |
         reinterpret_cast<uintptr_t>(boundary_value)) & 15u) return ULTRA_ERR_BAD_SHAPE;
    hipStream_t s = static_cast<hipStream_t>(stream);
    hipEvent_t ev_start = g_prof_start, ev_stop = g_prof_stop;
    g_prof_start = g_prof_stop = nullptr;
    if (ev_start != nullptr || ev_stop != nullptr) {
        hipStreamCaptureStatus cs = hipStreamCaptureStatusNone;
        HIP_TRY(hipStreamIsCapturing(s, &cs));
        if (cs != hipStreamCaptureStatusNone) ev_start = ev_stop = nullptr;
    }
    if (ev_start != nullptr) HIP_TRY(hipEventRecord(ev_start, s));
    {
        const long long n4 = (long long)n_dst * F / 4;
        const unsigned blocks = (unsigned)((n4 + 256 * 8 - 1) / (256 * 8) < 4096 ? (n4 + 256 * 8 - 1) / (256 * 8) : 4096);
        hipLaunchKernelGGL(zero_fill_kernel, dim3(blocks ? blocks : 1), dim3(256), 0, s, reinterpret_cast<qf4 *>(out), n4);
        HIP_TRY(hipGetLastError());
    }
    FrontierParams p{};
    p.src_ptr = src_ptr;
    p.dst = by_src->node_a;
    p.rel = by_src->rel;
    p.weight = by_src->weight;
    p.fwd_rank = fwd_rank;
    p.relation = relation;
    p.bnode = boundary_node;
    p.bvec = boundary_value;
    p.out = out;
    p.F = F;
    p.piece_len = (int)by_src->piece_len;
    p.n_rel = (int)n_rel;
    p.piece_shift = -1;
    for (int sh = 0; sh < 31; ++sh)
        if ((1LL << sh) == by_src->piece_len) p.piece_shift = sh;
    const size_t msg_bytes = (size_t)n_rel * kTile * sizeof(float);
    if (!g_force_general && n_rel > 0 && msg_bytes <= (size_t)kMaxLdsBytes) {
        p.slices = kFrontierLdsSlices;
        const int grid = (int)(F / 64) * p.slices;
        int rc = by_src->weight == nullptr
                     ? launch_with_lds(frontier_lds_kernel<true>, p, grid, msg_bytes, s, kFrontierLdsThreads)
                     : launch_with_lds(frontier_lds_kernel<false>, p, grid, msg_bytes, s, kFrontierLdsThreads);
        if (rc) return rc;
// ... 409 lines not shown
```

### ultra_torchdrug_amd/functional.py

```python
import collections

import torch

from . import _lib, _torch_ext
from .relcsr import RelCSR

__all__ = ["generalized_rspmm", "rspmm_forward", "rotate_rspmm", "rotate_rspmm_forward","first_layer_forward", "dense_layer_forward", "combine_forward", "combine", "linear_forward", "linear_supported", "score_all_entities", "relation_stack_inputs", "statistics", "bce_adversarial_loss", "candidate_tiles", "candidate_rows", "score_candidates", "RelCSR"]

_sparse_cache = collections.OrderedDict()
_SPARSE_CACHE_ENTRIES = 4


def accepts(tensor):
    return bool(tensor.is_cuda)


def _ops(sum, mul):
    if sum not in _lib.SUM_OPS:
        raise ValueError("Can't find a rspmm operator for sum=`%s` (expected add, min or max)" % sum)
    if mul not in _lib.MUL_OPS:
        raise ValueError("Can't find a rspmm operator for mul=`%s` (expected mul or add)" % mul)
    return _lib.SUM_OPS[sum], _lib.MUL_OPS[mul]


def _as_relcsr(sparse):
    if isinstance(sparse, RelCSR):
        return sparse, None
    if not isinstance(sparse, torch.Tensor) or not sparse.is_sparse:
        raise TypeError("sparse must be a 3-D torch sparse COO tensor or a RelCSR, got %s" % type(sparse).__name__)
    idx, val = sparse._indices(), sparse._values()
    key = (idx.data_ptr(), val.data_ptr(), idx._version, val._version, tuple(sparse.shape))
    hit = _sparse_cache.get(key)
    if hit is None:
        hit = (RelCSR.from_sparse(sparse), idx, val)
        _sparse_cache[key] = hit
        while len(_sparse_cache) > _SPARSE_CACHE_ENTRIES:
            _sparse_cache.popitem(last=False)
    else:
        _sparse_cache.move_to_end(key)
    return hit[0], (sparse if sparse.requires_grad else None)


def _check_dense(csr, relation, input, require_hip=True):
    n_dst, n_src, n_rel = csr.shape
    if input.dim() != 2 or relation.dim() != 2:
        raise RuntimeError("relation and input must be 2-D, got %s and %s" % (tuple(relation.shape), tuple(input.shape)))
    if input.shape[0] != n_src:
        raise RuntimeError("Expect input to have %d rows, but found %d" % (n_src, input.shape[0]))
    if relation.shape[0] != n_rel:
        raise RuntimeError("Expect relation to have %d rows, but found %d" % (n_rel, relation.shape[0]))
    if relation.shape[1] != input.shape[1]:
        raise RuntimeError("Expect relation and input to have the same width, but found %d and %d"
                           % (relation.shape[1], input.shape[1]))
    if input.dtype != torch.float32 or relation.dtype != torch.float32:
        raise RuntimeError("rspmm is fp32 only (TF32 is disabled in the reference, script/run_full.py:19-20)")
    if require_hip and (not input.is_cuda or not relation.is_cuda):
        raise RuntimeError("this operator of ultra_torchdrug_amd runs on an MI355X (HIP) device only; "
                           "got input on %s, relation on %s (only generalized_rspmm has CPU kernels)"
                           % (input.device, relation.device))
    if input.device != relation.device or input.device != csr.device:
        raise RuntimeError("sparse, relation and input must be on one device (%s, %s, %s)"
                           % (csr.device, relation.device, input.device))


def _stream():
    return torch.cuda.current_stream().cuda_stream


def _workspace(seg, F, device):
    n = seg.workspace_rows * F
    if n == 0:
        return None, 0
    ws = torch.empty(n, dtype=torch.float32, device=device)
    return ws, n * 4


def rspmm_forward(csr, relation, input, sum="add", mul="mul", add_rows=None, boundary=None):
    sum_op, mul_op = _ops(sum, mul)
    _check_dense(csr, relation, input)
    relation, input = relation.contiguous(), input.contiguous()
    F = input.shape[1]
    out = torch.empty(csr.shape[0], F, dtype=torch.float32, device=input.device)
    if add_rows is not None:
        add_rows = add_rows.contiguous()
        if add_rows.shape != out.shape or add_rows.dtype != torch.float32 or add_rows.device != out.device:
            raise RuntimeError("add_rows must be fp32 %s on %s" % (tuple(out.shape), out.device))
    if boundary is not None:
        if add_rows is not None:
            raise RuntimeError("give the boundary either dense (add_rows) or sparse (boundary), not both")
        b_node, b_value = boundary
        b_value = b_value.contiguous()
        if (b_node.dtype != torch.int32 or b_value.dtype != torch.float32 or b_node.dim() != 1 or b_value.dim() != 2
                or b_value.shape[0] != b_node.shape[0] or b_value.numel() != F or b_node.device != out.device
                or b_value.device != out.device or not b_node.is_contiguous()):
            raise RuntimeError("boundary must be (int32 (B,), fp32 (B, D)) with B * D == %d on %s" % (F, out.device))
    if out.numel() == 0:
        return out
    seg = csr.fwd
    if _torch_ext.binding() == "torch":
        b_node_, b_value_ = (boundary[0], b_value) if boundary is not None else (None, None)
        return _torch_ext.load().rspmm_plan_fwd(seg.plan_tensor, relation, input, add_rows, b_node_, b_value_,
                                                csr.shape[1], sum_op, mul_op)
    lib = _lib.load()
    ws, ws_bytes = _workspace(seg, F, input.device)
    if boundary is not None:
        with torch.cuda.device(input.device):
            _lib.check(lib.ultra_rspmm_forward_boundary_f32(
                seg.pointer, relation.data_ptr(), input.data_ptr(), b_node.data_ptr(), b_value.data_ptr(),
                b_value.shape[1], out.data_ptr(), ws.data_ptr() if ws is not None else None, ws_bytes, csr.shape[1],
                csr.shape[2], F, sum_op, mul_op, _stream()))
        return out
    with torch.cuda.device(input.device):
        _lib.check(lib.ultra_rspmm_forward_f32(
            seg.pointer, relation.data_ptr(), input.data_ptr(), add_rows.data_ptr() if add_rows is not None else None,
            out.data_ptr(), ws.data_ptr() if ws is not None else None, ws_bytes, csr.shape[1], csr.shape[2], F, sum_op,
            mul_op, _stream()))
    return out


def rspmm_forward_csr(row_ptr, src, rel, weight, relation, input, sum="add", mul="mul"):
    sum_op, mul_op = _ops(sum, mul)
    if input.dim() != 2 or relation.dim() != 2 or relation.shape[1] != input.shape[1]:
        raise RuntimeError("relation (R, F) and input (N_src, F) expected, got %s and %s"
                           % (tuple(relation.shape), tuple(input.shape)))
    tensors = [row_ptr, src, rel, relation, input] + ([weight] if weight is not None else [])
    if any(not t.is_cuda or t.device != input.device for t in tensors):
        raise RuntimeError("rspmm_forward_csr runs on an MI355X (HIP) device only. There is no CPU fallback.")
    if row_ptr.dtype != torch.int32 or src.dtype != torch.int32 or rel.dtype != torch.int32:
        raise RuntimeError("rspmm_forward_csr: row_ptr / src / rel must be int32")
    if input.dtype != torch.float32 or relation.dtype != torch.float32 or (weight is not None and weight.dtype != torch.float32):
        raise RuntimeError("rspmm is fp32 only (TF32 is disabled in the reference, script/run_full.py:19-20)")
    F = input.shape[1]
    if F % 4:
        raise RuntimeError("rspmm_forward_csr needs 16-byte rows (F % 4 == 0); use a RelCSR plan for other widths")
    n_rows, n_edges = row_ptr.numel() - 1, src.numel()
    relation, input = relation.contiguous(), input.contiguous()
    out = torch.empty(n_rows, F, dtype=torch.float32, device=input.device)
    if out.numel() == 0:
        return out
    lib = _lib.load()
    with torch.cuda.device(input.device):
        _lib.check(lib.ultra_rspmm_fwd_f32(
            row_ptr.contiguous().data_ptr(), src.contiguous().data_ptr(), rel.contiguous().data_ptr(),
            weight.contiguous().data_ptr() if weight is not None else None, relation.data_ptr(), input.data_ptr(),
            out.data_ptr(), n_rows, n_edges, relation.shape[0], F, sum_op, mul_op, _stream()))
    return out


def frontier_supported(sum, mul, F):
    return sum == "add" and mul == "mul" and F % 64 == 0


def rspmm_frontier(csr, relation, boundary):
    b_node, b_value = boundary
    b_value = b_value.contiguous()
    n_dst, n_src, n_rel = csr.shape
    F = b_value.numel()
    if relation.dim() != 2 or relation.shape != (n_rel, F) or relation.dtype != torch.float32 or not relation.is_cuda:
        raise RuntimeError("rspmm_frontier: relation must be fp32 (%d, %d) on the HIP device" % (n_rel, F))
    if (b_node.dtype != torch.int32 or b_node.dim() != 1 or b_value.dtype != torch.float32 or b_value.dim() != 2
# ... 91 lines not shown
    src_ptr, fwd_rank = csr.frontier_index
    run_prefix, max_runs = csr.frontier_runs
    update = torch.empty(n_dst, n_query, 64, dtype=torch.float32, device=dev)
    out = torch.empty(n_dst, n_query, 64, dtype=torch.float32, device=dev)
    row_list = torch.empty(n_query * (max_runs + 1), dtype=torch.int32, device=dev)
    list_offset = torch.empty(n_query + 1, dtype=torch.int32, device=dev)
    with torch.cuda.device(dev):
        _lib.check(lib.ultra_first_layer_sparse_train_f32(
            csr.by_src.pointer, src_ptr.data_ptr(), fwd_rank.data_ptr(), run_prefix.data_ptr(), relation.data_ptr(),
            b_node.data_ptr(), b_value.data_ptr(), n_query, weight.contiguous().data_ptr(), bias.contiguous().data_ptr(),
            ln_weight.contiguous().data_ptr() if ln_weight is not None else None,
            ln_bias.contiguous().data_ptr() if ln_weight is not None else None, float(ln_eps), int(bool(relu)), int(bool(shortcut)),
            update.data_ptr(), out.data_ptr(), row_list.data_ptr(), row_list.numel(), int(max_runs), list_offset.data_ptr(),
            n_dst, n_rel, _stream()))
    return update, out, row_list, list_offset[n_query:]


FUSED_LAYER = __import__("os").environ.get("ULTRA_FUSED_LAYER", "1") != "0"
FUSED_SCORE = __import__("os").environ.get("ULTRA_FUSED_SCORE", "1") != "0"


SECOND_LAYER_SOURCES = __import__("os").environ.get("ULTRA_SECOND_LAYER_SOURCES", "1") != "0"


def second_layer_sources(csr, row_list, list_count, n_query):
    if not SECOND_LAYER_SOURCES or not FUSED_LAYER:
        return None
    n_dst, n_src, n_rel = csr.shape
    plan = csr.fwd
    lib = _lib.load()
    if (n_dst != n_src or not lib.ultra_layer_forward_supported(plan.pointer, n_query, n_rel)
            or row_list.numel() * 64 > n_src or row_list.numel() + 1 >= n_src):
        return None
    dev = row_list.device
    E = plan.n_edges
    slack = plan.node_a.numel() - E
    sources = torch.empty(E + slack, dtype=torch.int32, device=dev)
    bitmap = torch.empty((n_src + 31) // 32, dtype=torch.int32, device=dev)
    c_node = torch.empty(1, dtype=torch.int32, device=dev)
    with torch.cuda.device(dev):
        _lib.check(lib.ultra_second_layer_sources(plan.node_a.data_ptr(), E, slack, row_list.data_ptr(), list_count.data_ptr(),
                                                  row_list.numel(), n_query, n_src, bitmap.data_ptr(), c_node.data_ptr(),
                                                  sources.data_ptr(), _stream()))
    return sources


def layer_forward(csr, relation, input, boundary, weight, bias, ln_weight=None, ln_bias=None, ln_eps=1e-5, relu=True,
                  shortcut=False, sources=None):
    if not FUSED_LAYER or input.dim() != 3 or input.shape[-1] != 64:
        return None
    n_dst, n_src, n_rel = csr.shape
    n_query = input.shape[1]
    lib = _lib.load()
    plan = csr.fwd
    if n_dst != n_src or input.shape[0] != n_src or not lib.ultra_layer_forward_supported(plan.pointer, n_query, n_rel):
        return None
    F = n_query * 64
    b_node, b_value = (None, None) if boundary is None else boundary
    tensors = [relation, input, weight, bias] + ([ln_weight, ln_bias] if ln_weight is not None else []) + ([b_value] if b_value is not None else [])
    if (ln_weight is not None and ln_bias is None) or any(t.numel() != 64 for t in tensors[3:4 + (2 if ln_weight is not None else 0)]):
        return None
    if (tuple(relation.shape) != (n_rel, F) or tuple(weight.shape) != (64, 128)
            or any(t.dtype != torch.float32 or not t.is_cuda or t.device != input.device for t in tensors)
            or (b_node is not None and (b_node.dtype != torch.int32 or tuple(b_node.shape) != (n_query,) or tuple(b_value.shape) != (n_query, 64)))):
        return None
    relation, input = relation.contiguous(), input.contiguous()
    out = torch.empty_like(input)
    if sources is not None:
        if sources.dtype != torch.int32 or sources.numel() != plan.node_a.numel() or sources.device != input.device:
            raise RuntimeError("layer_forward: sources must be second_layer_sources() of this plan")
        with torch.cuda.device(input.device):
            _lib.check(lib.ultra_layer_forward_sources_f32(
                plan.pointer, sources.data_ptr(), relation.data_ptr(), input.data_ptr(),
                b_node.contiguous().data_ptr() if b_node is not None else None,
                b_value.contiguous().data_ptr() if b_value is not None else None, n_query, weight.contiguous().data_ptr(),
                bias.contiguous().data_ptr(), ln_weight.contiguous().data_ptr() if ln_weight is not None else None,
                ln_bias.contiguous().data_ptr() if ln_weight is not None else None, float(ln_eps), int(bool(relu)), int(bool(shortcut)),
                out.data_ptr(), n_rel, _stream()))
        return out
    with torch.cuda.device(input.device):
        _lib.check(lib.ultra_layer_forward_f32(
            plan.pointer, relation.data_ptr(), input.data_ptr(), b_node.contiguous().data_ptr() if b_node is not None else None,
            b_value.contiguous().data_ptr() if b_value is not None else None, n_query, weight.contiguous().data_ptr(),
            bias.contiguous().data_ptr(), ln_weight.contiguous().data_ptr() if ln_weight is not None else None,
            ln_bias.contiguous().data_ptr() if ln_weight is not None else None, float(ln_eps), int(bool(relu)), int(bool(shortcut)),
            out.data_ptr(), n_rel, _stream()))
    return out


def layer_score_forward(csr, relation, input, boundary, weight, bias, ln_weight, ln_bias, ln_eps, relu, shortcut, query, w1, b1, w2,
                        b2):
    if not FUSED_LAYER or not FUSED_SCORE or input.dim() != 3 or input.shape[-1] != 64:
        return None
    n_dst, n_src, n_rel = csr.shape
    n_query = input.shape[1]
    lib = _lib.load()
    plan = csr.fwd
    if n_dst != n_src or input.shape[0] != n_src or not lib.ultra_layer_score_supported(plan.pointer, n_query, n_rel):
        return None
    F = n_query * 64
    b_node, b_value = (None, None) if boundary is None else boundary
    tensors = [relation, input, weight, bias, query, w1, b1, w2, b2] + ([ln_weight, ln_bias] if ln_weight is not None else []) \
        + ([b_value] if b_value is not None else [])
    if (ln_weight is not None and ln_bias is None) or bias.numel() != 64 or b1.numel() != 128 \
            or (ln_weight is not None and (ln_weight.numel() != 64 or ln_bias.numel() != 64)):
        return None
    if (tuple(relation.shape) != (n_rel, F) or tuple(weight.shape) != (64, 128) or tuple(w1.shape) != (128, 128) or w2.numel() != 128
            or b2.numel() != 1 or tuple(query.shape) != (n_query, 64)
            or any(t.dtype != torch.float32 or not t.is_cuda or t.device != input.device for t in tensors)
            or (b_node is not None and (b_node.dtype != torch.int32 or tuple(b_node.shape) != (n_query,) or tuple(b_value.shape) != (n_query, 64)))):
        return None
    relation, input = relation.contiguous(), input.contiguous()
    score = torch.empty(n_query, n_src, dtype=torch.float32, device=input.device)
    qbias = torch.empty(n_query, 128, dtype=torch.float32, device=input.device)
    with torch.cuda.device(input.device):
        _lib.check(lib.ultra_layer_score_forward_f32(
            plan.pointer, relation.data_ptr(), input.data_ptr(), b_node.contiguous().data_ptr() if b_node is not None else None,
            b_value.contiguous().data_ptr() if b_value is not None else None, n_query, weight.contiguous().data_ptr(),
            bias.contiguous().data_ptr(), ln_weight.contiguous().data_ptr() if ln_weight is not None else None,
            ln_bias.contiguous().data_ptr() if ln_weight is not None else None, float(ln_eps), int(bool(relu)), int(bool(shortcut)),
            query.contiguous().data_ptr(), w1.contiguous().data_ptr(), b1.contiguous().data_ptr(), w2.contiguous().data_ptr(),
            b2.contiguous().data_ptr(), qbias.data_ptr(), score.data_ptr(), n_rel, _stream()))
    return score


DENSE_LAYER = __import__("os").environ.get("ULTRA_DENSE_LAYER", "1") != "0"


def dense_layer_forward(csr, relation, input, boundary, weight, bias, ln_weight=None, ln_bias=None, ln_eps=1e-5, relu=True,
                        shortcut=False):
    if not DENSE_LAYER or not getattr(csr, "dense_form", False) or input.dim() != 3 or input.shape[-1] != 64:
        return None
    n, n_query = input.shape[0], input.shape[1]
    F = n_query * 64
    seg = csr.fwd
    lib = _lib.load()
    if seg.dense is None or csr.shape[0] != n or csr.shape[1] != n or csr.shape[2] != 4 or \
            not lib.ultra_dense_layer_supported(seg.pointer, n_query):
        return None
    b_node, b_value = boundary
    b_value = b_value.contiguous()
    tensors = [relation, input, b_value, weight, bias] + ([ln_weight, ln_bias] if ln_weight is not None else [])
    if (tuple(relation.shape) != (4, F) or tuple(b_value.shape) != (n_query, 64) or b_node.dtype != torch.int32
            or not b_node.is_contiguous() or tuple(weight.shape) != (64, 128)
            or any(t.dtype != torch.float32 or not t.is_cuda or t.device != input.device for t in tensors)
            or b_node.device != input.device or csr.device != input.device):
        raise RuntimeError("dense_layer_forward: input fp32 (N, Q, 64), relation fp32 (4, Q * 64), boundary (int32 (Q,), fp32 "
                           "(Q, 64)), a (64, 128) weight, all on one HIP device")
    relation, input = relation.contiguous(), input.contiguous()
    out = torch.empty_like(input)
    with torch.cuda.device(input.device):
        _lib.check(lib.ultra_dense_layer_forward_f32(
            seg.pointer, relation.data_ptr(), input.data_ptr(), b_node.data_ptr(), b_value.data_ptr(), n_query,
            weight.contiguous().data_ptr(), bias.contiguous().data_ptr(),
            ln_weight.contiguous().data_ptr() if ln_weight is not None else None,
            ln_bias.contiguous().data_ptr() if ln_weight is not None else None, float(ln_eps), int(bool(relu)), int(bool(shortcut)),
            out.data_ptr(), _stream()))
    return out


ACTIVE_ROW_BACKWARD = __import__("os").environ.get("ULTRA_ACTIVE_ROW_BACKWARD", "1") != "0"


BOUNDARY_DRELATION = __import__("os").environ.get("ULTRA_BOUNDARY_DRELATION", "1") != "0"


def rspmm_drelation_boundary(csr, input, output_grad, b_node):
    input, output_grad = input.contiguous(), output_grad.contiguous()
    dev, F = input.device, input.shape[1]
    n_dst, n_src, n_rel = csr.shape
    if (input.dtype != torch.float32 or output_grad.dtype != torch.float32 or not input.is_cuda or output_grad.device != dev
            or tuple(input.shape) != (n_src, F) or tuple(output_grad.shape) != (n_dst, F) or F % 64 != 0 or F == 0):
        raise RuntimeError("rspmm_drelation_boundary: fp32 device tensors (N_src, F) and (N_dst, F) with F a multiple of 64")
    if b_node.dtype != torch.int32 or not b_node.is_contiguous() or b_node.device != dev or tuple(b_node.shape) != (F // 64,):
        raise RuntimeError("rspmm_drelation_boundary: b_node must be contiguous int32 (%d,) on %s" % (F // 64, dev))
    items, src_ptr, src_relpos = csr.boundary_relation_index
    plan = csr.by_rel
    d_relation = torch.empty(n_rel, F, dtype=torch.float32, device=dev)
    n_ws = int(plan.n_pieces) * F
    ws = torch.empty(n_ws, dtype=torch.float32, device=dev) if n_ws else None
    lib = _lib.load()
    with torch.cuda.device(dev):
        _lib.check(lib.ultra_rspmm_drelation_boundary_f32(
            plan.pointer, items.data_ptr(), items.shape[0], src_ptr.data_ptr(), src_relpos.data_ptr(), b_node.data_ptr(),
            input.data_ptr(), output_grad.data_ptr(), d_relation.data_ptr(), ws.data_ptr() if ws is not None else None, n_ws * 4,
            n_src, n_rel, F, _stream()))
    return d_relation


def candidate_rows(t_index, n_node):
    if not ACTIVE_ROW_BACKWARD or not t_index.is_cuda or t_index.dtype != torch.int64 or t_index.dim() != 2:
        return None
    n_words = (int(n_node) + 31) // 32
    if n_words > 16384 or n_words == 0:
        return None
    t_index = t_index.contiguous()
    bits = torch.empty(t_index.shape[0], n_words, dtype=torch.int32, device=t_index.device)
    lib = _lib.load()
    with torch.cuda.device(t_index.device):
        _lib.check(lib.ultra_node_bitmap(t_index.data_ptr(), t_index.shape[0], t_index.shape[1], int(n_node), bits.data_ptr(),
                                         _stream()))
    return bits


def rspmm_backward(csr, relation, input, output, output_grad, sum="add", mul="mul", need_input=True,
                   need_relation=True, d_input_add=None, active_dst=None, active_src=None):
    sum_op, mul_op = _ops(sum, mul)
    relation, input, output_grad = relation.contiguous(), input.contiguous(), output_grad.contiguous()
    F = input.shape[1]
    dev = input.device
    if (ACTIVE_ROW_BACKWARD and sum == "add" and F % 64 == 0 and F > 0 and (need_input or need_relation)
            and (active_dst is not None or (active_src is not None and mul == "mul"))):
        n_tiles = F // 64
        if active_dst is not None and (active_dst.dtype != torch.int32 or not active_dst.is_contiguous() or active_dst.device != dev
                                       or tuple(active_dst.shape) != (n_tiles, (csr.shape[0] + 31) // 32)):
            raise RuntimeError("rspmm_backward: active_dst must be contiguous int32 (%d, %d) on %s"
                               % (n_tiles, (csr.shape[0] + 31) // 32, dev))
        if active_src is not None and (active_src.dtype != torch.int32 or not active_src.is_contiguous() or active_src.device != dev
                                       or tuple(active_src.shape) != (n_tiles,)):
            raise RuntimeError("rspmm_backward: active_src must be contiguous int32 (%d,) on %s" % (n_tiles, dev))
        if d_input_add is not None and (not need_input or not d_input_add.is_contiguous() or d_input_add.shape != input.shape
                                        or d_input_add.dtype != torch.float32):
            raise RuntimeError("d_input_add: contiguous fp32 tensor of input's shape, sum aggregation, with need_input")
        d_input = (d_input_add if d_input_add is not None else torch.empty_like(input)) if need_input else None
        d_relation = torch.empty_like(relation) if need_relation else None
        by_src = csr.by_src if need_input else None
        by_rel = csr.by_rel if need_relation else None
        lib = _lib.load()
        n_ws = max(by_src.workspace_rows if by_src is not None else 0, by_rel.workspace_rows if by_rel is not None else 0) * F
        ws = torch.empty(n_ws, dtype=torch.float32, device=dev) if n_ws else None
        with torch.cuda.device(dev):
            _lib.check(lib.ultra_rspmm_backward_active_f32(
                by_src.pointer if by_src is not None else None, by_rel.pointer if by_rel is not None else None,
                relation.data_ptr(), input.data_ptr(), output_grad.data_ptr(),
                d_input_add.data_ptr() if d_input_add is not None else None,
                d_input.data_ptr() if d_input is not None else None, d_relation.data_ptr() if d_relation is not None else None,
                ws.data_ptr() if ws is not None else None, n_ws * 4, csr.shape[1], csr.shape[0], csr.shape[2], F, mul_op,
                active_dst.data_ptr() if active_dst is not None else None, active_dst.shape[1] if active_dst is not None else 0,
                active_src.data_ptr() if (active_src is not None and mul == "mul") else None, _stream()))
        return d_input, d_relation
    if d_input_add is not None and (not need_input or sum != "add" or not d_input_add.is_contiguous()
                                    or d_input_add.shape != input.shape or d_input_add.dtype != torch.float32):
        raise RuntimeError("d_input_add: contiguous fp32 tensor of input's shape, sum aggregation, with need_input")
    d_input = (d_input_add if d_input_add is not None else torch.empty_like(input)) if need_input else None
    d_relation = torch.empty_like(relation) if need_relation else None
    if F == 0 or (not need_input and not need_relation):
        return d_input, d_relation
    by_src = csr.by_src if need_input else None
    by_rel = csr.by_rel if need_relation else None
    if _torch_ext.binding() == "torch":
        d_rel = _torch_ext.load().rspmm_plan_bwd(
            by_src.plan_tensor if by_src is not None else None, by_rel.plan_tensor if by_rel is not None else None,
            relation, input, output, output_grad, d_input, d_input_add is not None, csr.shape[1], csr.shape[0], sum_op, mul_op)
        return d_input, (d_rel if need_relation else None)
    lib = _lib.load()
    n_ws = max(by_src.workspace_rows if by_src is not None else 0, by_rel.workspace_rows if by_rel is not None else 0) * F
    ws = torch.empty(n_ws, dtype=torch.float32, device=dev) if n_ws else None
    with torch.cuda.device(dev):
        _lib.check(lib.ultra_rspmm_backward_accumulate_f32(
            by_src.pointer if by_src is not None else None, by_rel.pointer if by_rel is not None else None,
            relation.data_ptr(), input.data_ptr(), output.data_ptr() if output is not None else None,
            output_grad.data_ptr(), d_input_add.data_ptr() if d_input_add is not None else None,
            d_input.data_ptr() if d_input is not None else None,
            d_relation.data_ptr() if d_relation is not None else None, ws.data_ptr() if ws is not None else None,
            n_ws * 4, csr.shape[1], csr.shape[0], csr.shape[2], F, sum_op, mul_op, _stream()))
    return d_input, d_relation


def rspmm_backward_boundary_rows(csr, relation, output_grad, boundary_node, d_input, mul="mul"):
    _, mul_op = _ops("add", mul)
    n_query = boundary_node.shape[0]
    F = n_query * 64
    if (boundary_node.dtype != torch.int32 or not boundary_node.is_contiguous() or d_input.dtype != torch.float32
            or not d_input.is_contiguous() or tuple(d_input.shape) != (csr.shape[1], F) or not output_grad.is_contiguous()
            or tuple(output_grad.shape) != (csr.shape[0], F) or output_grad.dtype != torch.float32
            or tuple(relation.shape) != (csr.shape[2], F) or not relation.is_contiguous() or csr.shape[0] != csr.shape[1]):
        raise RuntimeError("rspmm_backward_boundary_rows: contiguous fp32 (N, Q * 64) gradients, int32 (Q,) nodes, a square adjacency")
    src_ptr, _ = csr.frontier_index
    lib = _lib.load()
    ws = torch.empty(max(int(lib.ultra_rspmm_backward_boundary_rows_workspace(n_query)) // 4, 1), dtype=torch.float32,
                     device=d_input.device)
    with torch.cuda.device(d_input.device):
        _lib.check(lib.ultra_rspmm_backward_boundary_rows_f32(
            csr.by_src.pointer, src_ptr.data_ptr(), relation.data_ptr(), output_grad.data_ptr(), boundary_node.data_ptr(),
            d_input.data_ptr(), ws.data_ptr(), ws.numel() * 4, csr.shape[1], n_query, F, mul_op, _stream()))
    return d_input


def rspmm_backward_weight(csr, relation, input, output, output_grad, sum="add", mul="mul"):
    sum_op, mul_op = _ops(sum, mul)
    relation, input, output_grad = relation.contiguous(), input.contiguous(), output_grad.contiguous()
    d_w = torch.zeros(csr.n_edges, dtype=torch.float32, device=input.device)
    if csr.n_edges == 0 or input.shape[1] == 0:
        return d_w
    lib = _lib.load()
    with torch.cuda.device(input.device):
        _lib.check(lib.ultra_rspmm_backward_weight_f32(
            csr.fwd.pointer, relation.data_ptr(), input.data_ptr(), output.data_ptr() if output is not None else None,
            output_grad.data_ptr(), d_w.data_ptr(), csr.shape[2], input.shape[1], sum_op, mul_op, _stream()))
    return d_w


def combine_forward(input, update, weight, bias, ln_weight=None, ln_bias=None, ln_eps=1e-5, relu=True, shortcut=False,
                    reuse_update=False, input_boundary=None, z_out=None):
    if input_boundary is not None:
        if input is not None:
# ... 877 lines not shown
```

### ultra_torchdrug_amd/rel_model.py

```python
import os
from collections.abc import Sequence

import torch
from torch import nn

from . import layer
from .graph import Graph


def construct_relation_graph(graph):
    graph = graph.undirected(add_inverse=True)
    device = graph.device
    n_rel, n_node = graph.num_relation, graph.num_node
    if graph.edge_list.is_cuda and 0 < n_rel <= 32768:
        from . import functional
        blocks = functional.relation_graph_blocks(graph.edge_list, n_node, n_rel)
        edges = []
        for etype in range(4):
            idx = blocks[etype].nonzero()
            edges.append(torch.cat([idx, torch.full((idx.shape[0], 1), etype, dtype=torch.long, device=device)], dim=1))
        return Graph(torch.cat(edges, dim=0), num_node=n_rel, num_relation=4)

    def incidence(col):
        pairs = graph.edge_list[:, [col, 2]].unique(dim=0)
        degree = torch.zeros(n_node, dtype=torch.long, device=device).index_add_(
            0, pairs[:, 0], torch.ones_like(pairs[:, 1]))
        assert not (degree[pairs[:, 0]] == 0).any()
        ones = torch.ones(pairs.shape[0], device=device)
        normalised_t = torch.sparse_coo_tensor(pairs.flip(1).t(), ones / degree[pairs[:, 0]], (n_rel, n_node))
        plain = torch.sparse_coo_tensor(pairs.t(), ones, (n_node, n_rel))
        return normalised_t, plain

    EhT, Eh = incidence(0)
    EtT, Et = incidence(1)
    blocks = [torch.sparse.mm(EhT, Eh), torch.sparse.mm(EtT, Et), torch.sparse.mm(EhT, Et), torch.sparse.mm(EtT, Eh)]
    edges = []
    for etype, block in enumerate(blocks):
        idx = block.coalesce().indices().t()
        edges.append(torch.cat([idx, torch.full((idx.shape[0], 1), etype, dtype=torch.long, device=device)], dim=1))
    return Graph(torch.cat(edges, dim=0), num_node=n_rel, num_relation=4)


TILED_TABLES_TRAIN = os.environ.get("ULTRA_TILED_TABLES_TRAIN", "1") != "0"


class _TiledTables(torch.autograd.Function):

    @staticmethod
    def forward(ctx, batch_size, *weights):
        n_rel, dim = weights[0].shape
        ctx.batch_size = batch_size
        tiled = torch.stack(weights).unsqueeze(2).expand(-1, -1, batch_size, -1).reshape(len(weights), n_rel, batch_size * dim)
        return tuple(tiled.unbind(0))

    @staticmethod
    def backward(ctx, *grads):
        live = next(g for g in grads if g is not None)
        dim = live.shape[1] // ctx.batch_size
        total = torch.stack([torch.zeros_like(live) if g is None else g for g in grads])
        total = total.view(len(grads), live.shape[0], ctx.batch_size, dim).sum(2)
        return (None,) + tuple(None if g is None else t for g, t in zip(grads, total.unbind(0)))


class CustomNBFNet(nn.Module):

    def __init__(self, input_dim, hidden_dims, num_relation=None, symmetric=False, message_func="distmult",
                 aggregate_func="pna", short_cut=False, layer_norm=False, activation="relu", concat_hidden=False,
                 num_mlp_layer=2, dependent=False, remove_one_hop=False, num_beam=10, path_topk=10,
                 separate_remove_one_hop=False):
        super().__init__()
        if not isinstance(hidden_dims, Sequence):
            hidden_dims = [hidden_dims]
        num_relation = 1 if num_relation is None else int(num_relation)
        self.dims = [input_dim] + list(hidden_dims)
        self.num_relation = num_relation
        self.symmetric = symmetric
        self.short_cut = short_cut
        self.concat_hidden = concat_hidden
        self.remove_one_hop = remove_one_hop
        self.layers = nn.ModuleList(
            layer.GeneralizedRelationalConvNBF(self.dims[i], self.dims[i + 1], num_relation, self.dims[0],
                                               message_func, aggregate_func, layer_norm, activation, dependent)
            for i in range(len(self.dims) - 1))
        feature_dim = hidden_dims[-1] * (len(hidden_dims) if concat_hidden else 1) + input_dim
        self.mlp = layer.MLP(feature_dim, [feature_dim] * (num_mlp_layer - 1) + [hidden_dims[-1]])

    def _tiled_tables(self, graph, batch_size):
        convs = list(self.layers)
        if not convs or any(conv.dependent for conv in convs):
            return None
        weights = [conv.relation.weight for conv in convs]
        if any(w.shape != weights[0].shape or not w.is_cuda for w in weights):
            return None
        if torch.is_grad_enabled():
            if not TILED_TABLES_TRAIN or any(w.dtype != torch.float32 for w in weights):
                return None
            return {id(conv): table for conv, table in zip(convs, _TiledTables.apply(batch_size, *weights))}
        n_rel, dim = weights[0].shape
        tiled = torch.stack(weights).unsqueeze(2).expand(-1, -1, batch_size, -1).reshape(len(convs), n_rel, batch_size * dim)
        return {id(conv): tiled[i] for i, conv in enumerate(convs)}

    def _run_layers(self, graph, boundary):
        graph.relation_tables = self._tiled_tables(graph, boundary.shape[1])
        layer_input = boundary
        for conv in self.layers:
            hidden = conv(graph, layer_input, shortcut=self.short_cut and conv.output_dim == layer_input.shape[-1],
                          input_is_boundary=layer_input is boundary)
            layer_input = hidden
        return layer_input

    def bellmanford(self, graph, h_index, separate_grad=False):
        dev = h_index.device
        query = torch.ones(h_index.shape[0], self.dims[0], device=dev)
        boundary = torch.zeros(graph.num_node, query.shape[1], device=dev)
        boundary[h_index] = 1.0
        graph.query = query.unsqueeze(0)
        graph.boundary = boundary.unsqueeze(1)
        graph.boundary_sparse = None
        return {"node_feature": self._run_layers(graph, boundary.unsqueeze(1)).squeeze(1)}

    def forward(self, graph, h_index, t_index=None, r_index=None, all_loss=None, metric=None):
        if not graph.num_relation:
            relation = torch.zeros(graph.num_edge, 1, dtype=torch.long, device=graph.device)
            graph = Graph(torch.cat([graph.edge_list[:, :2], relation], dim=-1), graph.edge_weight, graph.num_node, 1)
        return self.bellmanford(graph, h_index)["node_feature"]


class CustomNBFNetFull(CustomNBFNet):

    def __init__(self, learn_query=False, **kwargs):
        super().__init__(**kwargs)
        self.learn_query = learn_query
        if learn_query:
            self.learnable_q = nn.Embedding(1, self.dims[0])

    def _fast_bellmanford(self, graph, h_index):
        F = torch.nn.functional
        ops = layer.backend.get()
        if (not getattr(ops, "FAST_INFERENCE", False) or torch.is_grad_enabled() or self.learn_query or self.concat_hidden
                or not layer.FRONTIER_FIRST_LAYER or not ops.accepts(h_index) or not self.layers
                or graph.requires_grad):
            return None
        for conv in self.layers:
            ok = (isinstance(conv, layer.GeneralizedRelationalConvNBF) and not conv.dependent and conv.message_func == "distmult"
                  and conv.aggregate_func == "sum" and conv.input_dim == 64 and conv.output_dim == 64
                  and tuple(conv.linear.weight.shape) == (64, 128) and conv.linear.bias is not None
                  and (conv.activation is F.relu or not conv.activation) and conv.relation.weight.is_cuda
                  and conv.relation.weight.dtype == torch.float32 and conv.linear.weight.dtype == torch.float32
                  and (conv.layer_norm is None or (conv.layer_norm.elementwise_affine and conv.layer_norm.bias is not None)))
            if not ok:
                return None
            assert graph.num_relation == conv.num_relation
        n_query = h_index.shape[0]
        if not ops.frontier_supported("add", "mul", 64 * n_query):
            return None
        weights = [conv.relation.weight for conv in self.layers]
        if len(weights) > 8 or self.dims[0] != 64 or not n_query:
            return None
        tables, query, node32 = ops.relation_stack_inputs(weights, h_index)
        if not layer._frontier_tables_finite(tables[0]):
            return None
        boundary = (node32, query)
        csr = graph.relcsr
        n_node = graph.num_node
        hidden = None
        for i, conv in enumerate(self.layers):
            ln = conv.layer_norm
            args = (conv.linear.weight, conv.linear.bias, ln.weight if ln else None, ln.bias if ln else None,
                    ln.eps if ln else 1e-5, conv.activation is F.relu, self.short_cut)
            if i == 0:
                update = ops.rspmm_frontier(csr, tables[0], boundary).view(n_node, n_query, 64)
                hidden = ops.combine_forward(None, update, *args, reuse_update=True, input_boundary=boundary)
            else:
                fused = ops.dense_layer_forward(csr, tables[i], hidden, boundary, *args)
                if fused is not None:
                    hidden = fused
                    continue
                update = ops.rspmm_forward(csr, tables[i], hidden.flatten(1), "add", "mul", boundary=boundary)
                hidden = ops.combine_forward(hidden, update.view(n_node, n_query, 64), *args, reuse_update=True)
        return {"node_feature": hidden.transpose(1, 0)}

    def bellmanford(self, graph, h_index, separate_grad=False):
        fast = self._fast_bellmanford(graph, h_index)
        if fast is not None:
            return fast
        dev = h_index.device
        if self.learn_query:
            query = self.learnable_q.weight.expand(h_index.shape[0], self.dims[0])
        else:
            query = torch.ones(h_index.shape[0], self.dims[0], device=dev)
        index = h_index.unsqueeze(-1).expand_as(query)
        boundary = torch.zeros(graph.num_node, *query.shape, device=dev)
        boundary.scatter_add_(0, index.unsqueeze(0), query.unsqueeze(0))
        graph.query = query
        graph.boundary = boundary
        graph.boundary_sparse = (h_index.to(torch.int32), query)
        return {"node_feature": self._run_layers(graph, boundary).transpose(1, 0)}


class RelNBFNet(nn.Module):

    def __init__(self, input_dim, hidden, num_layers=6, input_type="ones", num_relation=None, **kwargs):
        super().__init__()
        self.input_dim = input_dim
        self.hidden_dim = hidden
        self.input_type = input_type
        self.num_relation = num_relation
        self.ablation_etypes = kwargs.get("ablation_etypes", False)
        self.model = CustomNBFNetFull(input_dim=input_dim, hidden_dims=[hidden] * num_layers,
                                      num_relation=4 if not self.ablation_etypes else None, aggregate_func="sum",
                                      layer_norm=True, short_cut=True, learn_query=kwargs.get("learn_query", False))
        if self.hidden_dim != self.input_dim:
            self.input_transform_linear = nn.Linear(self.input_dim, self.hidden_dim)

    def construct_relation_graph(self, graph):
        return construct_relation_graph(graph)

    def forward(self, graph, input, r_idx, all_loss=None, metric=None):
        assert input is None
        x = self.model(graph, h_index=r_idx)
        return {"graph_feature": None, "node_feature": x}


class RelationModelList(nn.ModuleList):

    def __init__(self, num_rel_models=1, num_relation=None, rel_model=None, **kwargs):
        super().__init__()
        self.num_rel_models = num_rel_models
        self.num_relation = num_relation
        cfg = dict(rel_model or {})
        cls = cfg.pop("class_str", "RelNBFNet")
        if cls != "RelNBFNet":
            raise ValueError("only RelNBFNet relation models are shipped, got `%s`" % cls)
        for _ in range(num_rel_models):
            self.append(RelNBFNet(**cfg, num_relation=num_relation))
```

Measured before the change: 43.87 billion.

## Fuse dense relation-graph first layer and pair row tiles in dense kernels

Adds a fused dense first-layer kernel for the relation graph that runs the boundary-only aggregation and the linear, layernorm and relu epilogue in one launch, replacing the frontier rspmm plus a separate combine. It also templates the dense row-sum and layer kernels on a row-tile count so that two 16-row adjacency tiles can share each gathered input load, which cuts repeated gather traffic. A host heuristic picks the tile count. Shared memory and register use grow with the paired tiles, which may lower occupancy.

```diff
diff --git a/include/ultra_rspmm.h b/include/ultra_rspmm.h
--- a/include/ultra_rspmm.h
+++ b/include/ultra_rspmm.h
@@ -275,6 +275,12 @@
                                   const float *bias, const float *ln_weight, const float *ln_bias, float ln_eps, int relu,
                                   int shortcut, float *out, void *stream);
 
+int ultra_dense_first_layer_supported(const ultra_segments *fwd, int64_t n_query);
+int ultra_dense_first_layer_forward_f32(const ultra_segments *fwd, const float *relation, const int32_t *boundary_node,
+                                        const float *boundary_value, int64_t n_query, const float *weight, const float *bias,
+                                        const float *ln_weight, const float *ln_bias, float ln_eps, int relu, int shortcut,
+                                        float *out, void *stream);
+
 int ultra_layer_forward_supported(const ultra_segments *fwd, int64_t n_query, int64_t n_rel);
 int ultra_layer_forward_f32(const ultra_segments *fwd, const float *relation, const float *input, const int32_t *boundary_node,
                             const float *boundary_value, int64_t n_query, const float *weight, const float *bias,
diff --git a/ultra_torchdrug_amd/_lib.py b/ultra_torchdrug_amd/_lib.py
--- a/ultra_torchdrug_amd/_lib.py
+++ b/ultra_torchdrug_amd/_lib.py
@@ -114,6 +114,8 @@
     "ultra_column_sum_f32",
     "ultra_dense_layer_supported",
     "ultra_dense_layer_forward_f32",
+    "ultra_dense_first_layer_supported",
+    "ultra_dense_first_layer_forward_f32",
     "ultra_layer_forward_supported",
     "ultra_layer_forward_f32",
     "ultra_second_layer_sources",
@@ -303,6 +305,10 @@
     lib.ultra_dense_layer_supported.argtypes = [seg, i64]
     lib.ultra_dense_layer_forward_f32.restype = i32
     lib.ultra_dense_layer_forward_f32.argtypes = [seg, vp, vp, vp, vp, i64, vp, vp, vp, vp, ctypes.c_float, i32, i32, vp, vp]
+    lib.ultra_dense_first_layer_supported.restype = i32
+    lib.ultra_dense_first_layer_supported.argtypes = [seg, i64]
+    lib.ultra_dense_first_layer_forward_f32.restype = i32
+    lib.ultra_dense_first_layer_forward_f32.argtypes = [seg, vp, vp, vp, i64, vp, vp, vp, vp, ctypes.c_float, i32, i32, vp, vp]
     lib.ultra_calibrate_gather_f32.restype = i32
     lib.ultra_calibrate_gather_f32.argtypes = [vp, i64, vp, i64, vp, ctypes.POINTER(i64), vp]
     lib.ultra_rspmm_rotate_forward_f32.restype = i32
diff --git a/ultra_torchdrug_amd/csrc/relgraph_dense.h b/ultra_torchdrug_amd/csrc/relgraph_dense.h
--- a/ultra_torchdrug_amd/csrc/relgraph_dense.h
+++ b/ultra_torchdrug_amd/csrc/relgraph_dense.h
@@ -28,6 +28,7 @@
 
 int persistent_cus(int *n_cu);
 bool wide_groups_forced();
+int dense_pairing_forced();
 
 bool dense_applies(const DenseCall &call);
 int dense_launch(const DenseCall &call, hipStream_t stream);
diff --git a/ultra_torchdrug_amd/csrc/relgraph_dense.hip b/ultra_torchdrug_amd/csrc/relgraph_dense.hip
--- a/ultra_torchdrug_amd/csrc/relgraph_dense.hip
+++ b/ultra_torchdrug_amd/csrc/relgraph_dense.hip
@@ -45,13 +45,15 @@
     int n_items, per_xcd;
 };
 
+template <int RT = 1>
 __device__ __forceinline__ bool dense_item(const DenseParams &p, int &vt, int &ct) {
     const int j = blockIdx.x / kXcd;
     const int item = (blockIdx.x % kXcd) * p.per_xcd + j;
     if (j >= p.per_xcd || item >= p.n_items) return false;
     const int n_qb = (p.n_ct + kDnWaves - 1) / kDnWaves;
-    vt = item / n_qb;
-    ct = (item - vt * n_qb) * kDnWaves + uniform((int)(threadIdx.x >> 6));
+    const int group = item / n_qb;
+    vt = group * RT;
+    ct = (item - group * n_qb) * kDnWaves + uniform((int)(threadIdx.x >> 6));
     return ct < p.n_ct;
 }
 
@@ -68,8 +70,8 @@
 #endif
 }
 
-template <int MUL, bool HAS_REL>
-__device__ __forceinline__ dn4 dense_rows_sum(const DenseParams &p, const int vt, const int ct, const int lane) {
+template <int MUL, bool HAS_REL, int RT>
+__device__ __forceinline__ void dense_rows_sum(const DenseParams &p, const int vt, const int ct, const int lane, dn4 (&acc)[RT]) {
     const int i = lane & 15, kq = lane >> 4;
     const long long F = p.F;
     const int col = ct * 16 + i;
@@ -79,16 +81,26 @@
     const __amdgpu_buffer_rsrc_t rsrc_x =
         __builtin_amdgcn_make_buffer_rsrc(const_cast<float *>(p.gather), 0, (int)((uint32_t)p.n_cols * row_bytes), 0x00020000);
     const uint32_t slab_words = (uint32_t)(p.cols_pad / 4) * 64u;
-    const __amdgpu_buffer_rsrc_t rsrc_a = __builtin_amdgcn_make_buffer_rsrc(
-        const_cast<uint32_t *>(p.adj + (long long)vt * slab_words), 0, (int)((slab_words + 4u * 64u) * 4u), 0x00020000);
+    __amdgpu_buffer_rsrc_t rsrc_a[RT];
+#pragma unroll
+    for (int t = 0; t < RT; ++t) {
+        const bool live = vt + t < p.n_vt;
+        rsrc_a[t] = __builtin_amdgcn_make_buffer_rsrc(const_cast<uint32_t *>(p.adj + (long long)(live ? vt + t : vt) * slab_words), 0,
+                                                      live ? (int)((slab_words + 4u * 64u) * 4u) : 0, 0x00020000);
+    }
     const uint32_t voff_x0 = (uint32_t)kq * row_bytes + (uint32_t)col * 4u, voff_a = (uint32_t)lane * 4u;
     const int pick[4] = {4 * i, 4 * (i + 16), 4 * (i + 32), 4 * (i + 48)};
 
-    auto load = [&](int u0, float (&x)[2], uint32_t (&a)[2]) {
+    auto load_x = [&](int u0, float (&x)[2]) {
+#pragma unroll
+        for (int h = 0; h < 2; ++h)
+            x[h] = __builtin_bit_cast(float, __builtin_amdgcn_raw_buffer_load_b32(rsrc_x, voff_x0 + (uint32_t)(u0 + 4 * h) * row_bytes, 0, 0));
+    };
+    auto load_a = [&](int u0, uint32_t (&a)[RT][2]) {
 #pragma unroll
         for (int h = 0; h < 2; ++h) {
-            x[h] = __builtin_bit_cast(float, __builtin_amdgcn_raw_buffer_load_b32(rsrc_x, voff_x0 + (uint32_t)(u0 + 4 * h) * row_bytes, 0, 0));
-            a[h] = __builtin_amdgcn_raw_buffer_load_b32(rsrc_a, voff_a, (uint32_t)(u0 / 4 + h) * 256u, 0);
+#pragma unroll
+            for (int t = 0; t < RT; ++t) a[t][h] = __builtin_amdgcn_raw_buffer_load_b32(rsrc_a[t], voff_a, (uint32_t)(u0 / 4 + h) * 256u, 0);
         }
     };
     auto spread = [&](const float (&x)[2], float (&xs)[kDnU]) {
@@ -103,7 +115,8 @@
 #endif
         }
     };
-    dn4 acc = {0.0f, 0.0f, 0.0f, 0.0f};
+#pragma unroll
+    for (int t = 0; t < RT; ++t) acc[t] = dn4{0.0f, 0.0f, 0.0f, 0.0f};
     auto message = [&](float xv) -> float {
 #if ULTRA_DN_VARIANT >= 3
         return xv;
@@ -111,44 +124,70 @@
         if constexpr (!HAS_REL) return xv;
         return (MUL == ULTRA_MUL_MUL) ? relv * xv : relv + xv;
     };
-    auto compute = [&](const float (&xs)[kDnU], const uint32_t (&a)[2]) {
-        acc = __builtin_amdgcn_mfma_f32_16x16x4f32(entry<0>(a[0]), message(xs[0]), acc, 0, 0, 0);
-        acc = __builtin_amdgcn_mfma_f32_16x16x4f32(entry<1>(a[0]), message(xs[1]), acc, 0, 0, 0);
-        acc = __builtin_amdgcn_mfma_f32_16x16x4f32(entry<2>(a[0]), message(xs[2]), acc, 0, 0, 0);
-        acc = __builtin_amdgcn_mfma_f32_16x16x4f32(entry<3>(a[0]), message(xs[3]), acc, 0, 0, 0);
-        acc = __builtin_amdgcn_mfma_f32_16x16x4f32(entry<0>(a[1]), message(xs[4]), acc, 0, 0, 0);
-        acc = __builtin_amdgcn_mfma_f32_16x16x4f32(entry<1>(a[1]), message(xs[5]), acc, 0, 0, 0);
-        acc = __builtin_amdgcn_mfma_f32_16x16x4f32(entry<2>(a[1]), message(xs[6]), acc, 0, 0, 0);
-        acc = __builtin_amdgcn_mfma_f32_16x16x4f32(entry<3>(a[1]), message(xs[7]), acc, 0, 0, 0);
+    auto compute = [&](const float (&xs)[kDnU], const uint32_t (&a)[RT][2]) {
+        float m[kDnU];
+#pragma unroll
+        for (int j = 0; j < kDnU; ++j) m[j] = message(xs[j]);
+#pragma unroll
+        for (int h = 0; h < 2; ++h) {
+#pragma unroll
+            for (int t = 0; t < RT; ++t) acc[t] = __builtin_amdgcn_mfma_f32_16x16x4f32(entry<0>(a[t][h]), m[4 * h + 0], acc[t], 0, 0, 0);
+#pragma unroll
+            for (int t = 0; t < RT; ++t) acc[t] = __builtin_amdgcn_mfma_f32_16x16x4f32(entry<1>(a[t][h]), m[4 * h + 1], acc[t], 0, 0, 0);
+#pragma unroll
+            for (int t = 0; t < RT; ++t) acc[t] = __builtin_amdgcn_mfma_f32_16x16x4f32(entry<2>(a[t][h]), m[4 * h + 2], acc[t], 0, 0, 0);
+#pragma unroll
+            for (int t = 0; t < RT; ++t) acc[t] = __builtin_amdgcn_mfma_f32_16x16x4f32(entry<3>(a[t][h]), m[4 * h + 3], acc[t], 0, 0, 0);
+        }
     };
-    float x0[2], x1[2], s0[kDnU], s1[kDnU];
-    uint32_t a0[2], a1[2], c0[2], c1[2];
-    load(0, x0, a0);
-    load(kDnU, x1, a1);
-    spread(x0, s0);
-    c0[0] = a0[0]; c0[1] = a0[1];
-    for (int u0 = 0; u0 < p.cols_pad; u0 += 2 * kDnU) {
-        load(u0 + 2 * kDnU, x0, a0);
-        spread(x1, s1);
-        c1[0] = a1[0]; c1[1] = a1[1];
-        compute(s0, c0);
-        load(u0 + 3 * kDnU, x1, a1);
+    if constexpr (RT == 1) {
+        float x0[2], x1[2], s0[kDnU], s1[kDnU];
+        uint32_t a0[RT][2], a1[RT][2], c0[RT][2], c1[RT][2];
+        load_x(0, x0); load_a(0, a0);
+        load_x(kDnU, x1); load_a(kDnU, a1);
         spread(x0, s0);
-        c0[0] = a0[0]; c0[1] = a0[1];
-        compute(s1, c1);
-    }
-    return acc;
-}
-
-template <int MUL, bool HAS_REL>
+        c0[0][0] = a0[0][0]; c0[0][1] = a0[0][1];
+        for (int u0 = 0; u0 < p.cols_pad; u0 += 2 * kDnU) {
+            load_x(u0 + 2 * kDnU, x0); load_a(u0 + 2 * kDnU, a0);
+            spread(x1, s1);
+            c1[0][0] = a1[0][0]; c1[0][1] = a1[0][1];
+            compute(s0, c0);
+            load_x(u0 + 3 * kDnU, x1); load_a(u0 + 3 * kDnU, a1);
+            spread(x0, s0);
+            c0[0][0] = a0[0][0]; c0[0][1] = a0[0][1];
+            compute(s1, c1);
+        }
+    } else {
+        float x0[2], x1[2], s0[kDnU], s1[kDnU];
+        uint32_t a0[RT][2], a1[RT][2];
+        load_x(0, x0); load_a(0, a0);
+        load_x(kDnU, x1);
+        spread(x0, s0);
+        for (int u0 = 0; u0 < p.cols_pad; u0 += 2 * kDnU) {
+            load_x(u0 + 2 * kDnU, x0); load_a(u0 + kDnU, a1);
+            spread(x1, s1);
+            __builtin_amdgcn_sched_barrier(0);
+            compute(s0, a0);
+            __builtin_amdgcn_sched_barrier(0);
+            load_x(u0 + 3 * kDnU, x1); load_a(u0 + 2 * kDnU, a0);
+            spread(x0, s0);
+            __builtin_amdgcn_sched_barrier(0);
+            compute(s1, a1);
+            __builtin_amdgcn_sched_barrier(0);
+        }
+    }
+}
+
+template <int MUL, bool HAS_REL, int RT>
 __global__ __launch_bounds__(kDnWaves * 64) void dense_rows_kernel(const DenseParams p) {
     int vt, ct;
-    if (!dense_item(p, vt, ct)) return;
+    if (!dense_item<RT>(p, vt, ct)) return;
     const int lane = threadIdx.x & 63;
     const int i = lane & 15, kq = lane >> 4;
     const long long F = p.F;
     const int col = ct * 16 + i;
-    const dn4 acc = dense_rows_sum<MUL, HAS_REL>(p, vt, ct, lane);
+    dn4 acc[RT];
+    dense_rows_sum<MUL, HAS_REL, RT>(p, vt, ct, lane, acc);
 
     int b_node = -1;
     float b_val = 0.0f;
@@ -157,13 +196,16 @@
         b_val = p.bvec[col];
     }
 #pragma unroll
-    for (int r = 0; r < 4; ++r) {
-        const int row = vt * 16 + 4 * kq + r;
-        if (row < p.n_rows) {
-            float v = acc[r];
-            if (p.add_rows != nullptr) v = v + p.add_rows[(long long)row * F + col];
-            else if (p.bnode != nullptr) v = v + (row == b_node ? b_val : 0.0f);
-            p.out[(long long)row * F + col] = v;
+    for (int t = 0; t < RT; ++t) {
+#pragma unroll
+        for (int r = 0; r < 4; ++r) {
+            const int row = (vt + t) * 16 + 4 * kq + r;
+            if (row < p.n_rows) {
+                float v = acc[t][r];
+                if (p.add_rows != nullptr) v = v + p.add_rows[(long long)row * F + col];
+                else if (p.bnode != nullptr) v = v + (row == b_node ? b_val : 0.0f);
+                p.out[(long long)row * F + col] = v;
+            }
         }
     }
 }
@@ -177,78 +219,142 @@
     float *out;
 };
 constexpr int kDlStride = 68;
-
+constexpr int kDlTile = 16 * kDlStride;
+
+__device__ __forceinline__ void dense_layer_weights(const DenseLayerParams &q, const int wave, const int lane, float (&wf)[32]) {
+    const int i = lane & 15, kq = lane >> 4;
+    const float *wrow = q.weight + (long long)(16 * wave + i) * 128 + 64 * (kq & 1) + (kq >> 1);
+#pragma unroll
+    for (int j = 0; j < 32; ++j) wf[j] = wrow[2 * j];
+}
+
+template <int RT>
+__device__ __forceinline__ void dense_layer_finish(const DenseLayerParams &q, const int vt, const int ct, const int lane,
+                                                   const dn4 (&acc)[RT], const float (&wf)[32], const float bias, float *t_in,
+                                                   float *t_up, float *t_z) {
+    const DenseParams &p = q.d;
+    const int wave = ct & 3;
+    const int i = lane & 15, kq = lane >> 4;
+    const long long F = p.F;
+    const int col = ct * 16 + i;
+    {
+        const int b_node = p.bnode[col / 64];
+        const float b_val = p.bvec[col];
+#pragma unroll
+        for (int t = 0; t < RT; ++t) {
+#pragma unroll
+            for (int r = 0; r < 4; ++r) {
+                const int row = (vt + t) * 16 + 4 * kq + r;
+                t_up[t * kDlTile + (4 * kq + r) * kDlStride + 16 * wave + i] = acc[t][r] + (row == b_node ? b_val : 0.0f);
+            }
+        }
+    }
+    __syncthreads();
+    dn4 z[RT];
+#pragma unroll
+    for (int t = 0; t < RT; ++t) z[t] = dn4{bias, bias, bias, bias};
+    {
+        const float *src = ((kq & 1) ? t_up : t_in) + i * kDlStride + (kq >> 1);
+#pragma unroll
+        for (int j = 0; j < 32; ++j) {
+#pragma unroll
+            for (int t = 0; t < RT; ++t) z[t] = __builtin_amdgcn_mfma_f32_16x16x4f32(src[t * kDlTile + 2 * j], wf[j], z[t], 0, 0, 0);
+        }
+    }
+#pragma unroll
+    for (int t = 0; t < RT; ++t) {
+#pragma unroll
+        for (int r = 0; r < 4; ++r) t_z[t * kDlTile + (4 * kq + r) * kDlStride + 16 * wave + i] = z[t][r];
+    }
+    __syncthreads();
+    const int lrow = 4 * wave + kq;
+#pragma unroll
+    for (int t = 0; t < RT; ++t) {
+        const float *zr = t_z + t * kDlTile + lrow * kDlStride;
+        dn4 v = *reinterpret_cast<const dn4 *>(zr + 4 * i);
+        if (q.gamma != nullptr) {
+            const int half = (i >> 3) & 1;
+            float s = 0.0f;
+            if ((i & 7) == 0)
+                for (int c = 0; c < 32; ++c) s = s + zr[32 * half + c];
+            const float s0 = __shfl(s, 16 * kq, 64), s1 = __shfl(s, 16 * kq + 8, 64);
+            const float mean = (s0 + s1) * (1.0f / 64.0f);
+            float ss = 0.0f;
+            if ((i & 7) == 0)
+                for (int c = 0; c < 32; ++c) { const float dlt = zr[32 * half + c] - mean; ss = ss + dlt * dlt; }
+            const float q0 = __shfl(ss, 16 * kq, 64), q1 = __shfl(ss, 16 * kq + 8, 64);
+            const float var = (q0 + q1) * (1.0f / 64.0f);
+            const float inv = 1.0f / sqrtf(var + q.eps);
+            const dn4 g = *reinterpret_cast<const dn4 *>(q.gamma + 4 * i), b = *reinterpret_cast<const dn4 *>(q.beta + 4 * i);
+            v.x = ((v.x - mean) * inv) * g.x + b.x; v.y = ((v.y - mean) * inv) * g.y + b.y;
+            v.z = ((v.z - mean) * inv) * g.z + b.z; v.w = ((v.w - mean) * inv) * g.w + b.w;
+        }
+        if (q.relu) {
+            v.x = !(v.x <= 0.0f) ? v.x : 0.0f; v.y = !(v.y <= 0.0f) ? v.y : 0.0f; v.z = !(v.z <= 0.0f) ? v.z : 0.0f; v.w = !(v.w <= 0.0f) ? v.w : 0.0f;
+        }
+        if (q.shortcut) {
+            const dn4 x = *reinterpret_cast<const dn4 *>(t_in + t * kDlTile + lrow * kDlStride + 4 * i);
+            v.x = v.x + x.x; v.y = v.y + x.y; v.z = v.z + x.z; v.w = v.w + x.w;
+        }
+        const int row = (vt + t) * 16 + lrow;
+        if (row < p.n_rows) *reinterpret_cast<dn4 *>(q.out + (long long)row * F + (ct & ~3) * 16 + 4 * i) = v;
+    }
+}
+
+template <int RT>
 __global__ __launch_bounds__(kDnWaves * 64) void dense_layer_kernel(const DenseLayerParams q) {
     const DenseParams &p = q.d;
-    __shared__ __attribute__((aligned(16))) float t_in[16 * kDlStride], t_up[16 * kDlStride], t_z[16 * kDlStride];
+    __shared__ __attribute__((aligned(16))) float t_in[RT * kDlTile], t_up[RT * kDlTile], t_z[RT * kDlTile];
     int vt, ct;
-    if (!dense_item(p, vt, ct)) return;
+    if (!dense_item<RT>(p, vt, ct)) return;
+    const int lane = threadIdx.x & 63, wave = ct & 3;
+    const int i = lane & 15, kq = lane >> 4;
+    const long long F = p.F;
+    float wf[32];
+    dense_layer_weights(q, wave, lane, wf);
+    const float bias = q.bias[16 * wave + i];
+#pragma unroll
+    for (int t = 0; t < RT; ++t) {
+        const int row = (vt + t) * 16 + 4 * wave + kq;
+        dn4 v = {0.0f, 0.0f, 0.0f, 0.0f};
+        if (row < p.n_rows) v = *reinterpret_cast<const dn4 *>(p.gather + (long long)row * F + (ct & ~3) * 16 + 4 * i);
+        *reinterpret_cast<dn4 *>(t_in + t * kDlTile + (4 * wave + kq) * kDlStride + 4 * i) = v;
+    }
+    dn4 acc[RT];
+    dense_rows_sum<ULTRA_MUL_MUL, true, RT>(p, vt, ct, lane, acc);
+    dense_layer_finish<RT>(q, vt, ct, lane, acc, wf, bias, t_in, t_up, t_z);
+}
+
+__global__ __launch_bounds__(kDnWaves * 64) void dense_first_layer_kernel(const DenseLayerParams q) {
+    const DenseParams &p = q.d;
+    __shared__ __attribute__((aligned(16))) float t_in[kDlTile], t_up[kDlTile], t_z[kDlTile];
+    int vt, ct;
+    if (!dense_item<1>(p, vt, ct)) return;
     const int lane = threadIdx.x & 63, wave = ct & 3;
     const int i = lane & 15, kq = lane >> 4;
     const long long F = p.F;
     const int col = ct * 16 + i;
     float wf[32];
-    {
-        const float *wrow = q.weight + (long long)(16 * wave + i) * 128 + 64 * (kq & 1) + (kq >> 1);
-#pragma unroll
-        for (int j = 0; j < 32; ++j) wf[j] = wrow[2 * j];
-    }
+    dense_layer_weights(q, wave, lane, wf);
     const float bias = q.bias[16 * wave + i];
+    const int s = uniform(p.bnode[col / 64]);
+    const bool live = s >= 0 && s < p.n_rows;
     {
         const int row = vt * 16 + 4 * wave + kq;
         dn4 v = {0.0f, 0.0f, 0.0f, 0.0f};
-        if (row < p.n_rows) v = *reinterpret_cast<const dn4 *>(p.gather + (long long)row * F + (ct & ~3) * 16 + 4 * i);
+        if (row == s && live) v = *reinterpret_cast<const dn4 *>(p.bvec + (ct & ~3) * 16 + 4 * i);
         *reinterpret_cast<dn4 *>(t_in + (4 * wave + kq) * kDlStride + 4 * i) = v;
     }
-    const dn4 acc = dense_rows_sum<ULTRA_MUL_MUL, true>(p, vt, ct, lane);
-    {
-        const int b_node = p.bnode[col / 64];
-        const float b_val = p.bvec[col];
-#pragma unroll
-        for (int r = 0; r < 4; ++r) {
-            const int row = vt * 16 + 4 * kq + r;
-            t_up[(4 * kq + r) * kDlStride + 16 * wave + i] = acc[r] + (row == b_node ? b_val : 0.0f);
-        }
-    }
-    __syncthreads();
-    dn4 z = {bias, bias, bias, bias};
-    {
-        const float *src = ((kq & 1) ? t_up : t_in) + i * kDlStride + (kq >> 1);
-#pragma unroll
-        for (int j = 0; j < 32; ++j) z = __builtin_amdgcn_mfma_f32_16x16x4f32(src[2 * j], wf[j], z, 0, 0, 0);
-    }
-#pragma unroll
-    for (int r = 0; r < 4; ++r) t_z[(4 * kq + r) * kDlStride + 16 * wave + i] = z[r];
-    __syncthreads();
-    const int lrow = 4 * wave + kq;
-    const float *zr = t_z + lrow * kDlStride;
-    dn4 v = *reinterpret_cast<const dn4 *>(zr + 4 * i);
-    if (q.gamma != nullptr) {
-        const int half = (i >> 3) & 1;
-        float s = 0.0f;
-        if ((i & 7) == 0)
-            for (int c = 0; c < 32; ++c) s = s + zr[32 * half + c];
-        const float s0 = __shfl(s, 16 * kq, 64), s1 = __shfl(s, 16 * kq + 8, 64);
-        const float mean = (s0 + s1) * (1.0f / 64.0f);
-        float ss = 0.0f;
-        if ((i & 7) == 0)
-            for (int c = 0; c < 32; ++c) { const float dlt = zr[32 * half + c] - mean; ss = ss + dlt * dlt; }
-        const float q0 = __shfl(ss, 16 * kq, 64), q1 = __shfl(ss, 16 * kq + 8, 64);
-        const float var = (q0 + q1) * (1.0f / 64.0f);
-        const float inv = 1.0f / sqrtf(var + q.eps);
-        const dn4 g = *reinterpret_cast<const dn4 *>(q.gamma + 4 * i), b = *reinterpret_cast<const dn4 *>(q.beta + 4 * i);
-        v.x = ((v.x - mean) * inv) * g.x + b.x; v.y = ((v.y - mean) * inv) * g.y + b.y;
-        v.z = ((v.z - mean) * inv) * g.z + b.z; v.w = ((v.w - mean) * inv) * g.w + b.w;
-    }
-    if (q.relu) {
-        v.x = !(v.x <= 0.0f) ? v.x : 0.0f; v.y = !(v.y <= 0.0f) ? v.y : 0.0f; v.z = !(v.z <= 0.0f) ? v.z : 0.0f; v.w = !(v.w <= 0.0f) ? v.w : 0.0f;
-    }
-    if (q.shortcut) {
-        const dn4 x = *reinterpret_cast<const dn4 *>(t_in + lrow * kDlStride + 4 * i);
-        v.x = v.x + x.x; v.y = v.y + x.y; v.z = v.z + x.z; v.w = v.w + x.w;
-    }
-    const int row = vt * 16 + lrow;
-    if (row < p.n_rows) *reinterpret_cast<dn4 *>(q.out + (long long)row * F + (ct & ~3) * 16 + 4 * i) = v;
+    const uint32_t slab_words = (uint32_t)(p.cols_pad / 4) * 64u;
+    const __amdgpu_buffer_rsrc_t rsrc_a = __builtin_amdgcn_make_buffer_rsrc(
+        const_cast<uint32_t *>(p.adj + (long long)vt * slab_words), 0, (int)(slab_words * 4u), 0x00020000);
+    const uint32_t word = __builtin_amdgcn_raw_buffer_load_b32(rsrc_a, (uint32_t)lane * 4u, (uint32_t)(live ? s >> 2 : 0) * 256u, 0);
+    const float a = live ? (float)((word >> (8 * (s & 3))) & 0xffu) : 0.0f;
+    const float relv = p.relation[(long long)kq * F + col];
+    const float xv = p.bvec[col];
+    dn4 acc[1] = {dn4{0.0f, 0.0f, 0.0f, 0.0f}};
+    acc[0] = __builtin_amdgcn_mfma_f32_16x16x4f32(a, relv * xv, acc[0], 0, 0, 0);
+    dense_layer_finish<1>(q, vt, ct, lane, acc, wf, bias, t_in, t_up, t_z);
 }
 
 __global__ __launch_bounds__(kDnWaves * 64) void dense_drel_kernel(const DenseParams p) {
@@ -367,6 +473,20 @@
     return (int)((n_cols + round - 1) / round * round);
 }
 inline long long dense_slack_bytes(int kind) { return kind == 0 ? 2 * kDnU * 64 : 2 * 256; }
+
+int dense_row_tiles(int n_vt, int n_qb) {
+    const int forced = ultra_detail::dense_pairing_forced();
+    if (forced == 1 || n_vt < 2) return 1;
+    if (forced == 2) return 2;
+    int n_cu = 0;
+    if (ultra_detail::persistent_cus(&n_cu) != ULTRA_OK || n_cu <= 0) return 1;
+    return ((n_vt + 1) / 2) * n_qb >= n_cu ? 2 : 1;
+}
+
+inline void dense_grid(DenseParams &d, int n_qb, int rt) {
+    d.n_items = ((d.n_vt + rt - 1) / rt) * n_qb;
+    d.per_xcd = (d.n_items + kXcd - 1) / kXcd;
+}
 
 }
 
@@ -408,8 +528,8 @@
     q.n_ct = (int)(F / 16);
     q.cols_pad = dense_cols_pad(seg->dense_cols, c.kind == KIND_DREL ? 1 : 0);
     const int n_qb = (q.n_ct + kDnWaves - 1) / kDnWaves;
-    q.n_items = q.n_vt * n_qb;
-    q.per_xcd = (q.n_items + kXcd - 1) / kXcd;
+    const int rt = c.kind == KIND_DREL ? 1 : dense_row_tiles(q.n_vt, n_qb);
+    dense_grid(q, n_qb, rt);
     const dim3 grid((unsigned)(q.per_xcd * kXcd)), block(kDnWaves * 64);
     if (c.kind == KIND_DREL) {
         hipLaunchKernelGGL(dense_drel_kernel, grid, block, 0, stream, q);
@@ -417,12 +537,15 @@
         const long long n = 4 * F;
         hipLaunchKernelGGL(dense_drel_reduce_kernel, dim3((unsigned)((n + 255) / 256)), dim3(256), 0, stream,
                            static_cast<const float *>(c.workspace), c.out, F, q.n_vt);
+    } else if (c.mul_op == ULTRA_MUL_MUL) {
+        if (rt == 2) hipLaunchKernelGGL((dense_rows_kernel<ULTRA_MUL_MUL, true, 2>), grid, block, 0, stream, q);
+        else hipLaunchKernelGGL((dense_rows_kernel<ULTRA_MUL_MUL, true, 1>), grid, block, 0, stream, q);
     } else if (c.kind == KIND_FWD) {
-        if (c.mul_op == ULTRA_MUL_MUL) hipLaunchKernelGGL((dense_rows_kernel<ULTRA_MUL_MUL, true>), grid, block, 0, stream, q);
-        else hipLaunchKernelGGL((dense_rows_kernel<ULTRA_MUL_ADD, true>), grid, block, 0, stream, q);
+        if (rt == 2) hipLaunchKernelGGL((dense_rows_kernel<ULTRA_MUL_ADD, true, 2>), grid, block, 0, stream, q);
+        else hipLaunchKernelGGL((dense_rows_kernel<ULTRA_MUL_ADD, true, 1>), grid, block, 0, stream, q);
     } else {
-        if (c.mul_op == ULTRA_MUL_MUL) hipLaunchKernelGGL((dense_rows_kernel<ULTRA_MUL_MUL, true>), grid, block, 0, stream, q);
-        else hipLaunchKernelGGL((dense_rows_kernel<ULTRA_MUL_ADD, false>), grid, block, 0, stream, q);
+        if (rt == 2) hipLaunchKernelGGL((dense_rows_kernel<ULTRA_MUL_ADD, false, 2>), grid, block, 0, stream, q);
+        else hipLaunchKernelGGL((dense_rows_kernel<ULTRA_MUL_ADD, false, 1>), grid, block, 0, stream, q);
     }
     HIP_TRY(hipGetLastError());
     return ULTRA_OK;
@@ -460,6 +583,31 @@
         ids = nxt;
     }
     out[wave * 64 + lane] = acc;
+}
+
+int dense_layer_params(const ultra_segments *fwd, const float *relation, const float *input, const int32_t *boundary_node,
+                              const float *boundary_value, int64_t n_query, const float *weight, const float *bias,
+                              const float *ln_weight, const float *ln_bias, float ln_eps, int relu, int shortcut, float *out,
+                              bool first, DenseLayerParams &q) {
+    if (fwd != nullptr && (fwd->struct_bytes != (uint32_t)sizeof(ultra_segments) || fwd->abi_version != (uint32_t)ULTRA_RSPMM_ABI_VERSION))
+        return ULTRA_ERR_ABI;
+    if (!ultra_dense_layer_supported(fwd, n_query)) return ULTRA_ERR_BAD_SHAPE;
+    if (relation == nullptr || (!first && input == nullptr) || boundary_node == nullptr || boundary_value == nullptr ||
+        weight == nullptr || bias == nullptr || out == nullptr)
+        return ULTRA_ERR_NULL_POINTER;
+    if (ln_weight != nullptr && ln_bias == nullptr) return ULTRA_ERR_NULL_POINTER;
+    if (!first && out == input) return ULTRA_ERR_BAD_SHAPE;
+    if ((reinterpret_cast<uintptr_t>(out) | reinterpret_cast<uintptr_t>(input) | reinterpret_cast<uintptr_t>(ln_weight) |
+         reinterpret_cast<uintptr_t>(ln_bias) | (first ? reinterpret_cast<uintptr_t>(boundary_value) : 0)) & 15u)
+        return ULTRA_ERR_BAD_SHAPE;
+    DenseParams &d = q.d;
+    const long long F = n_query * 64;
+    d.adj = fwd->dense; d.relation = relation; d.gather = input; d.bnode = boundary_node; d.bvec = boundary_value; d.bdim = 64;
+    d.F = F; d.n_rows = (int)fwd->dense_rows; d.n_cols = (int)fwd->dense_cols; d.n_vt = (int)((fwd->dense_rows + 15) / 16);
+    d.n_ct = (int)(F / 16); d.cols_pad = dense_cols_pad(fwd->dense_cols, 0);
+    q.weight = weight; q.bias = bias; q.gamma = ln_weight; q.beta = ln_bias; q.eps = ln_eps; q.relu = relu; q.shortcut = shortcut;
+    q.out = out;
+    return ULTRA_OK;
 }
 
 }
@@ -510,27 +658,37 @@
                                   const int32_t *boundary_node, const float *boundary_value, int64_t n_query, const float *weight,
                                   const float *bias, const float *ln_weight, const float *ln_bias, float ln_eps, int relu,
                                   int shortcut, float *out, void *stream) {
-    if (fwd != nullptr && (fwd->struct_bytes != (uint32_t)sizeof(ultra_segments) || fwd->abi_version != (uint32_t)ULTRA_RSPMM_ABI_VERSION))
-        return ULTRA_ERR_ABI;
-    if (!ultra_dense_layer_supported(fwd, n_query)) return ULTRA_ERR_BAD_SHAPE;
-    if (relation == nullptr || input == nullptr || boundary_node == nullptr || boundary_value == nullptr || weight == nullptr ||
-        bias == nullptr || out == nullptr)
-        return ULTRA_ERR_NULL_POINTER;
-    if (ln_weight != nullptr && ln_bias == nullptr) return ULTRA_ERR_NULL_POINTER;
-    if (out == input) return ULTRA_ERR_BAD_SHAPE;
-    if ((reinterpret_cast<uintptr_t>(out) | reinterpret_cast<uintptr_t>(input) | reinterpret_cast<uintptr_t>(ln_weight) |
-         reinterpret_cast<uintptr_t>(ln_bias)) & 15u)
-        return ULTRA_ERR_BAD_SHAPE;
     DenseLayerParams q{};
+    const int rc = dense_layer_params(fwd, relation, input, boundary_node, boundary_value, n_query, weight, bias, ln_weight, ln_bias,
+                                      ln_eps, relu, shortcut, out, false, q);
+    if (rc) return rc;
     DenseParams &d = q.d;
-    const long long F = n_query * 64;
-    d.adj = fwd->dense; d.relation = relation; d.gather = input; d.bnode = boundary_node; d.bvec = boundary_value; d.bdim = 64;
-    d.F = F; d.n_rows = (int)fwd->dense_rows; d.n_cols = (int)fwd->dense_cols; d.n_vt = (int)((fwd->dense_rows + 15) / 16);
-    d.n_ct = (int)(F / 16); d.cols_pad = dense_cols_pad(fwd->dense_cols, 0);
-    d.n_items = d.n_vt * (d.n_ct / kDnWaves); d.per_xcd = (d.n_items + kXcd - 1) / kXcd;
-    q.weight = weight; q.bias = bias; q.gamma = ln_weight; q.beta = ln_bias; q.eps = ln_eps; q.relu = relu; q.shortcut = shortcut;
-    q.out = out;
-    hipLaunchKernelGGL(dense_layer_kernel, dim3((unsigned)(d.per_xcd * kXcd)), dim3(kDnWaves * 64), 0, static_cast<hipStream_t>(stream), q);
+    const int n_qb = d.n_ct / kDnWaves;
+    const int rt = dense_row_tiles(d.n_vt, n_qb);
+    dense_grid(d, n_qb, rt);
+    const dim3 grid((unsigned)(d.per_xcd * kXcd)), block(kDnWaves * 64);
+    if (rt == 2) hipLaunchKernelGGL(dense_layer_kernel<2>, grid, block, 0, static_cast<hipStream_t>(stream), q);
+    else hipLaunchKernelGGL(dense_layer_kernel<1>, grid, block, 0, static_cast<hipStream_t>(stream), q);
+    HIP_TRY(hipGetLastError());
+    return ULTRA_OK;
+}
+
+int ultra_dense_first_layer_supported(const ultra_segments *fwd, int64_t n_query) {
+    return (ultra_detail::dense_pairing_forced() != 1 && ultra_dense_layer_supported(fwd, n_query)) ? 1 : 0;
+}
+
+int ultra_dense_first_layer_forward_f32(const ultra_segments *fwd, const float *relation, const int32_t *boundary_node,
+                                        const float *boundary_value, int64_t n_query, const float *weight, const float *bias,
+                                        const float *ln_weight, const float *ln_bias, float ln_eps, int relu, int shortcut,
+                                        float *out, void *stream) {
+    DenseLayerParams q{};
+    const int rc = dense_layer_params(fwd, relation, nullptr, boundary_node, boundary_value, n_query, weight, bias, ln_weight,
+                                      ln_bias, ln_eps, relu, shortcut, out, true, q);
+    if (rc) return rc;
+    DenseParams &d = q.d;
+    dense_grid(d, d.n_ct / kDnWaves, 1);
+    hipLaunchKernelGGL(dense_first_layer_kernel, dim3((unsigned)(d.per_xcd * kXcd)), dim3(kDnWaves * 64), 0,
+                       static_cast<hipStream_t>(stream), q);
     HIP_TRY(hipGetLastError());
     return ULTRA_OK;
 }
diff --git a/ultra_torchdrug_amd/csrc/rspmm_kernels.hip b/ultra_torchdrug_amd/csrc/rspmm_kernels.hip
--- a/ultra_torchdrug_amd/csrc/rspmm_kernels.hip
+++ b/ultra_torchdrug_amd/csrc/rspmm_kernels.hip
@@ -839,6 +839,7 @@
 bool g_no_quad = false;
 bool g_wide_groups = false;
 bool g_no_dead_words = false;
+int g_dense_pairing = 0;
 #ifndef ULTRA_QUAD_U
 #define ULTRA_QUAD_U 8
 #endif
@@ -1393,6 +1394,7 @@
     return ULTRA_OK;
 }
 bool wide_groups_forced() { return g_wide_groups; }
+int dense_pairing_forced() { return g_dense_pairing; }
 }
 
 extern "C" {
@@ -1447,6 +1449,7 @@
     g_no_concurrent_tiles = (on & 32) != 0;
     g_no_dead_words = (on & 128) != 0;
     g_no_dense = (on & 64) != 0;
+    g_dense_pairing = (on & 256) ? 1 : (on & 512) ? 2 : 0;
     return ULTRA_OK;
 }
 
diff --git a/ultra_torchdrug_amd/functional.py b/ultra_torchdrug_amd/functional.py
--- a/ultra_torchdrug_amd/functional.py
+++ b/ultra_torchdrug_amd/functional.py
@@ -5,7 +5,7 @@
 from . import _lib, _torch_ext
 from .relcsr import RelCSR
 
-__all__ = ["generalized_rspmm", "rspmm_forward", "rotate_rspmm", "rotate_rspmm_forward","first_layer_forward", "dense_layer_forward", "combine_forward", "combine", "linear_forward", "linear_supported", "score_all_entities", "relation_stack_inputs", "statistics", "bce_adversarial_loss", "candidate_tiles", "candidate_rows", "score_candidates", "RelCSR"]
+__all__ = ["generalized_rspmm", "rspmm_forward", "rotate_rspmm", "rotate_rspmm_forward","first_layer_forward", "dense_layer_forward", "dense_first_layer_forward", "combine_forward", "combine", "linear_forward", "linear_supported", "score_all_entities", "relation_stack_inputs", "statistics", "bce_adversarial_loss", "candidate_tiles", "candidate_rows", "score_candidates", "RelCSR"]
 
 _sparse_cache = collections.OrderedDict()
 _SPARSE_CACHE_ENTRIES = 4
@@ -403,6 +403,40 @@
     with torch.cuda.device(input.device):
         _lib.check(lib.ultra_dense_layer_forward_f32(
             seg.pointer, relation.data_ptr(), input.data_ptr(), b_node.data_ptr(), b_value.data_ptr(), n_query,
+            weight.contiguous().data_ptr(), bias.contiguous().data_ptr(),
+            ln_weight.contiguous().data_ptr() if ln_weight is not None else None,
+            ln_bias.contiguous().data_ptr() if ln_weight is not None else None, float(ln_eps), int(bool(relu)), int(bool(shortcut)),
+            out.data_ptr(), _stream()))
+    return out
+
+
+def dense_first_layer_forward(csr, relation, boundary, weight, bias, ln_weight=None, ln_bias=None, ln_eps=1e-5, relu=True,
+                              shortcut=False):
+    if not DENSE_LAYER or not getattr(csr, "dense_form", False):
+        return None
+    b_node, b_value = boundary
+    n, n_query = csr.shape[0], b_node.shape[0]
+    F = n_query * 64
+    seg = csr.fwd
+    lib = _lib.load()
+    if seg.dense is None or csr.shape[1] != n or csr.shape[2] != 4 or not n_query or \
+            not lib.ultra_dense_first_layer_supported(seg.pointer, n_query):
+        return None
+    b_value = b_value.contiguous()
+    if b_value.data_ptr() % 16:
+        b_value = b_value.clone()
+    tensors = [relation, b_value, weight, bias] + ([ln_weight, ln_bias] if ln_weight is not None else [])
+    if (tuple(relation.shape) != (4, F) or tuple(b_value.shape) != (n_query, 64) or b_node.dtype != torch.int32
+            or b_node.dim() != 1 or not b_node.is_contiguous() or tuple(weight.shape) != (64, 128)
+            or any(t.dtype != torch.float32 or not t.is_cuda or t.device != relation.device for t in tensors)
+            or b_node.device != relation.device or csr.device != relation.device):
+        raise RuntimeError("dense_first_layer_forward: relation fp32 (4, Q * 64), boundary (int32 (Q,), fp32 (Q, 64)), a "
+                           "(64, 128) weight, all on one HIP device")
+    relation = relation.contiguous()
+    out = torch.empty(n, n_query, 64, dtype=torch.float32, device=relation.device)
+    with torch.cuda.device(relation.device):
+        _lib.check(lib.ultra_dense_first_layer_forward_f32(
+            seg.pointer, relation.data_ptr(), b_node.data_ptr(), b_value.data_ptr(), n_query,
             weight.contiguous().data_ptr(), bias.contiguous().data_ptr(),
             ln_weight.contiguous().data_ptr() if ln_weight is not None else None,
             ln_bias.contiguous().data_ptr() if ln_weight is not None else None, float(ln_eps), int(bool(relu)), int(bool(shortcut)),
diff --git a/ultra_torchdrug_amd/rel_model.py b/ultra_torchdrug_amd/rel_model.py
--- a/ultra_torchdrug_amd/rel_model.py
+++ b/ultra_torchdrug_amd/rel_model.py
@@ -169,6 +169,9 @@
             args = (conv.linear.weight, conv.linear.bias, ln.weight if ln else None, ln.bias if ln else None,
                     ln.eps if ln else 1e-5, conv.activation is F.relu, self.short_cut)
             if i == 0:
+                hidden = ops.dense_first_layer_forward(csr, tables[0], boundary, *args)
+                if hidden is not None:
+                    continue
                 update = ops.rspmm_frontier(csr, tables[0], boundary).view(n_node, n_query, 64)
                 hidden = ops.combine_forward(None, update, *args, reuse_update=True, input_boundary=boundary)
             else:
```

Result: no change. 44.24 billion (median of 6 runs) (+0.8%).
